# RashmikaDushan/MocapV2

Measured on AMD Instinct MI355X. Metric: frames/sec (6-cam 1080p), higher is better.
Workload: dtype u8+int64+f64; 1 GPU; 6-camera 1920x1080 synthetic IR frames, 8 markers (BASELINE.json configs[1]); cameras=6, width=1920, height=1080, markers=8, distortion=mild, frames_resident_in_hbm=True, batches_in_flight=3, resident_batches=3, status_ok=True, input=gray frames, parallelism=single launch, time-major

## Files before the change

### mocapv2_amd/csrc/abi_blob.hip

```cpp
#include "ctx.h"

static_assert(sizeof(mocap_contour) == sizeof(ContourRec), "debug record layout");

struct ScanTurn { std::mutex mu; hipEvent_t done = nullptr; bool have = false; };
static ScanTurn g_scan_turn[64];

extern "C" {

static int check_frames(mocap_ctx* c, const void* frames, int n_images, int cam_mod, int slot_base, size_t image_stride, int pitch)
{
    if (!c || !frames) return fail(MOCAP_E_INVALID, "null argument");
    if (n_images < 1) return fail(MOCAP_E_INVALID, "n_images = %d", n_images);
    if (cam_mod < 1 || slot_base < 0 || slot_base + cam_mod > c->n_slots)
        return fail(MOCAP_E_INVALID, "slots %d..%d not in 0..%d", slot_base, slot_base + cam_mod - 1, c->n_slots - 1);
    if (pitch < c->W) return fail(MOCAP_E_INVALID, "pitch %d < width %d", pitch, c->W);
    if (n_images > 1 && image_stride < (size_t)pitch * (c->H - 1) + c->W) return fail(MOCAP_E_INVALID, "image_stride too small");
    for (int s = slot_base; s < slot_base + cam_mod; s++)
        if (c->slot_state[s] == 0) return fail(MOCAP_E_STATE, "mocap_set_undistort was not called for slot %d", s);
    return 0;
}


static int excess_base(int thr_mul, int sel)
{
    int c = sel ? thr_mul - 67 : thr_mul - 154;
    if (c > thr_mul - 1) c = thr_mul - 1;
    if (c > 254) c = 254;
    return c < 0 ? 0 : c;
}

static int ensure_gray_scratch(mocap_ctx* c, size_t bytes)
{
    if (bytes <= c->gray_scratch.n) return 0;
    std::lock_guard<std::mutex> lk(c->mu);
    return c->gray_scratch.reserve(bytes);
}

static int threshold_mul(const mocap_ctx* c)
{
    const double ft = floor(c->prm.thresh);
    return ft < -1.0 ? 0 : (ft > 255.0 ? 256 : (int)ft + 1);
}

static FilterArgs filter_args(const mocap_ctx* c, const void* src, size_t image_stride, int pitch, uint32_t* mask, uint32_t* cells,
                              int slot_base, int cam_mod, int n_images, int thr_mul)
{
    const Tiling tl = tiling(c);
    FilterArgs a{};
    a.src = (const uint8_t*)src; a.image_stride = image_stride; a.pitch = pitch; a.H = c->H; a.W = c->W;
    a.mask = mask; a.words_per_row = c->wpr; a.cam_mod = cam_mod; a.cells = cells;
    a.n_images = n_images; a.n_steps = (n_images + cam_mod - 1) / cam_mod;
    a.thr_mul = thr_mul;
    a.n_strips = tl.n_strips; a.rows_per_chunk = tl.rows; a.n_cgroups = tl.n_cgroups;
    a.pipelined = c->W >= 4 && (c->W & 3) == 0 && c->H >= 2;
    if (slot_base >= 0) {
        a.map = slot_map(c, slot_base); a.mapw = slot_mapw(c, slot_base); a.map4 = slot_map4(c, slot_base);
        a.rowbox = c->rowbox ? c->rowbox + (size_t)slot_base * c->H * tl.n_strips : nullptr;
    }
    return a;
}

struct Batch {
    int n_images, cam_mod, slot_base;
    size_t image_stride; int pitch;
    uint32_t* mask; uint32_t* cells;
    bool own_mask;
    hipStream_t s;
};

static void read_probe(mocap_ctx* c, int thr_mul)
{
    if (!c->probe_pending || hipEventQuery(c->probe_ev) != hipSuccess) return;
    unsigned long long n_cur = 0, n_alt = 0;
    for (int i = 0; i < 128; i++) { n_cur += c->probe_host[PROBE_STRIDE * i]; n_alt += c->probe_host[PROBE_STRIDE * i + 1]; }
    if (c->tune.probe_debug) fprintf(stderr, "[probe] base %d: %llu hot cells, alternative %d: %llu\n", excess_base(thr_mul, c->base_sel), n_cur, excess_base(thr_mul, c->base_sel ^ 1), n_alt);
    const unsigned long long n_lo = c->base_sel == 0 ? n_cur : n_alt, n_hi = c->base_sel == 0 ? n_alt : n_cur;
    c->base_sel = (n_lo * 4 <= n_hi * 5) ? 0 : 1;
    const unsigned long long n_now = c->base_sel == 0 ? n_lo : n_hi;
    c->hot_dense = c->probe_images > 0 && n_now > 400ull * (unsigned long long)c->probe_images;
    c->probe_pending = false;
}

struct ScanBounds {
    int thr_mul;
    int fixed_base;
    int base, base_alt;
    int allow, allow_cut1, allow_cut2, allow_alt;
};
static ScanBounds scan_bounds(const mocap_ctx* c, int slot_base, int cam_mod, int thr_mul)
{
    ScanBounds b{thr_mul, c->tune.excess_base, 0, 0, -1, -1, -1, -1};
    if (b.fixed_base >= 0) { if (b.fixed_base > thr_mul - 1) b.fixed_base = thr_mul - 1; if (b.fixed_base > 254) b.fixed_base = 254; if (b.fixed_base < 0) b.fixed_base = 0; }
    b.base = b.fixed_base >= 0 ? b.fixed_base : excess_base(thr_mul, c->base_sel);
    b.base_alt = excess_base(thr_mul, c->base_sel ^ 1);
    long long wmax = 0;
    bool ok = true;
    for (int sl = slot_base; sl < slot_base + cam_mod; sl++) {
        if (c->slot_wmax[sl] == 0) ok = false;
        wmax = c->slot_wmax[sl] > wmax ? c->slot_wmax[sl] : wmax;
    }
    auto t5 = [](int n) { return (n - 1 < 2 ? n - 1 : 2) + 1; };
    auto t5full = [](int n) { return n < 5 ? n : 5; };
    const long long per_tap = 1024LL * (2LL * thr_mul - 2LL * b.base - 1), per_tap_alt = 1024LL * (2LL * thr_mul - 2LL * b.base_alt - 1);
    if (!c->tile_rows || !c->tile_cols || !c->reach || !c->cflags) ok = false;
    if (ok && wmax > 0 && per_tap > 0) {
        b.allow = (int)((per_tap * t5full(c->W) * t5full(c->H) - 1) / wmax);
        const long long taps1 = t5(c->W) * t5full(c->H) < t5full(c->W) * t5(c->H) ? t5(c->W) * t5full(c->H) : t5full(c->W) * t5(c->H);
        b.allow_cut1 = (int)((per_tap * taps1 - 1) / wmax);
        b.allow_cut2 = (int)((per_tap * t5(c->W) * t5(c->H) - 1) / wmax);
        if (per_tap_alt > 0) b.allow_alt = (int)((per_tap_alt * t5full(c->W) * t5full(c->H) - 1) / wmax);
    }
    if (!c->tune.skip_dark) b.allow = -1;
    return b;
}

struct FilterPath {
    bool remap;
    bool compact;
    bool rows_staged;
    bool direct;
    bool bayer;
    uint64_t remap_bits;
    int rows_dw;
    const void* frames;
    BayerArgs bl;
};
static int choose_path(mocap_ctx* c, const Batch& bt, const void* frames, const BayerArgs* bayer, int allow, FilterPath& p)
{
    p = FilterPath{};
    p.compact = c->W >= 8 && bt.cam_mod <= 64;
    for (int sl = bt.slot_base; sl < bt.slot_base + bt.cam_mod; sl++) {
        if (c->slot_state[sl] == 2) { p.remap = true; if (sl - bt.slot_base < 64) p.remap_bits |= 1ull << (sl - bt.slot_base); }
        if (c->slot_state[sl] == 2 && !c->slot_compact[sl]) p.compact = false;
    }
    if (c->tune.general_filter) p.compact = false;
    p.rows_staged = p.remap && c->tune.rows_staged && c->map4 && c->rowbox && (c->W & 15) == 0 && c->H >= 2;
    for (int sl = bt.slot_base; sl < bt.slot_base + bt.cam_mod; sl++)
        if (!c->slot_compact[sl]) p.rows_staged = false;
    p.rows_dw = c->tune.rows_stage_dw < 0 || c->tune.rows_stage_dw > rows_stage_dwords() ? rows_stage_dwords() : c->tune.rows_stage_dw;
    if (allow < 0 && !c->tune.dense_boxes) p.compact = false;
    p.frames = frames;
    p.bayer = bayer != nullptr;
    if (bayer) p.bl = *bayer;
    if (bayer && !bayer->dst) {
        p.direct = p.compact && allow >= 0 && bt.own_mask && bayer_scan_direct(p.bl);
        if (!p.direct) {
            const size_t bytes = (size_t)(bt.n_images - 1) * bt.image_stride + (size_t)(c->H - 1) * bt.pitch + c->W;
            TRY(ensure_gray_scratch(c, bytes));
            p.bl.dst = c->gray_scratch;
        }
        p.frames = p.direct ? (const void*)p.bl.src : (const void*)p.bl.dst;
    }
    return 0;
}

static int filter_dense(mocap_ctx* c, const Batch& bt, const FilterPath& p, int thr_mul)
{
    FilterArgs a = filter_args(c, p.frames, bt.image_stride, bt.pitch, bt.mask, bt.cells, bt.slot_base, bt.cam_mod, bt.n_images, thr_mul);
    if (!c->tune.remap_pipeline) a.pipelined = 0;
    a.staged = p.rows_staged; a.stage_dw = p.rows_dw;
    if (p.bayer) { launch_bayer_gray(p.bl, bt.s); HIP_TRY(hipGetLastError()); }
    if (bt.own_mask) c->mask_dirty = true;
    EvPair ev; bool on;
    prof_begin(c, bt.s, ev, on);
    launch_filter_mask(a, p.remap, bt.s);
    prof_end(c, PROF_FILTER, bt.s, ev, on);
    HIP_TRY(hipGetLastError());
    return 0;
}

static BoxArgs box_args(const mocap_ctx* c, const Batch& bt, const FilterPath& p, const ScanBounds& sb)
{
    const Tiling tl = tiling(c);
    BoxArgs a{};
    a.src = (const uint8_t*)p.frames; a.image_stride = bt.image_stride; a.pitch = bt.pitch; a.H = c->H; a.W = c->W;
    a.mask = bt.mask; a.words_per_row = c->wpr; a.cells = bt.cells;
    a.map4 = slot_map4(c, bt.slot_base);
    a.srcbox = c->srcbox ? c->srcbox + (size_t)bt.slot_base * source_cells(c) : nullptr;
    a.remap_bits = p.remap_bits;
    a.cam_mod = bt.cam_mod; a.n_images = bt.n_images; a.n_steps = (bt.n_images + bt.cam_mod - 1) / bt.cam_mod;
    a.thr_mul = sb.thr_mul;
    a.rows_per_chunk = tl.rows; a.n_strips = tl.n_strips; a.n_chunks = tl.n_cgroups * 4;
    const size_t tr_words = c->mask_images * cells_per_image(c) * 4;
    a.tile_rows = c->tile_rows + (c->tile_rows_flip ? tr_words : 0);
    a.tile_rows_next = c->tile_rows + (c->tile_rows_flip ? 0 : tr_words);
    a.n_clear = c->tile_rows_hold[c->tile_rows_flip ^ 1];
    a.tile_cols = c->tile_cols + (c->tile_rows_flip ? tr_words / 4 : 0);
    a.tile_cols_next = c->tile_cols + (c->tile_rows_flip ? 0 : tr_words / 4);
    a.wide_split = c->tune.wide_split == 2 || (c->tune.wide_split == 1 && !c->hot_dense);
    a.cluster = c->tune.cluster;
    a.cur_box = bt.own_mask ? c->cur_box : c->cur_box_ext;
    a.items = c->items; a.n_items = c->n_items; a.cap_items = (uint32_t)c->items.n;
    a.dense = sb.allow < 0;
    a.wide_tiles = c->wide_tiles; a.cap_wide = (uint32_t)c->wide_tiles.n; a.wide_quads_remap = c->tune.wide_quads_remap; a.wide_quads_identity = c->tune.wide_quads_identity;
    a.wide_bands = c->tune.wide_bands;
    if (c->W < 4 || p.direct) a.wide_tiles = nullptr;
    a.bayer = p.direct ? p.bl : BayerArgs{};
    a.stage_bytes = c->tune.box_stage_bytes;
    a.prio = c->tune.box_prio;
    a.ext_mask = bt.own_mask ? 0 : 1;
    return a;
}

static BrightArgs bright_args(const mocap_ctx* c, const Batch& bt, const FilterPath& p, const ScanBounds& sb, uint32_t* tile_rows, uint32_t* tile_cols,
                              bool scan_zeroes)
{
    const Tiling tl = tiling(c);
    uint64_t ncx64 = (uint64_t)((c->W + 7) / 8);
    const uint64_t ncells = ncx64 * (uint64_t)((c->H + 7) / 8);
    int wide = (c->W % 16 == 0) && (bt.pitch % 16 == 0) && (bt.image_stride % 16 == 0) && (((uintptr_t)p.frames & 15) == 0) && ncx64 >= 4;
    if (wide && ncells * (ncx64 / 2) >= (1ull << 32)) wide = 0;
    if (!c->tune.scan_wide) wide = 0;
    if (wide) ncx64 /= 2;
    const uint32_t ncx_magic = (ncx64 > 1 && ncells * ncx64 < (1ull << 32)) ? (uint32_t)(((1ull << 32) + ncx64 - 1) / ncx64) : 0u;
    BrightArgs b{(const uint8_t*)p.frames, bt.image_stride, bt.pitch, c->H, c->W, bt.n_images, bt.cam_mod, ncx_magic, wide, sb.base, sb.allow / 4, sb.allow_cut1 / 4, sb.allow_cut2 / 4,
                 c->reach + (size_t)bt.slot_base * source_cells(c), c->cflags + (size_t)bt.slot_base * source_cells(c),
                 tile_rows, tl.n_cgroups * 4, tl.n_strips, (uint32_t)(((1u << 23) + tl.rows - 1) / tl.rows),
                 bt.mask, bt.own_mask ? 0 : (size_t)bt.n_images * mask_image_words(c->H, c->wpr), ((uintptr_t)bt.mask & 15) == 0, nullptr, sb.base_alt, sb.allow_alt / 4, 0};
    b.prio = c->tune.scan_prio;
    b.max_blocks = c->tune.scan_blocks_per_cu * c->n_cu; b.blocks_x = 0;
    b.zero_counters = scan_zeroes ? c->n_items.p : nullptr;
    b.block_ctr = c->n_items + 160;
    b.slices = c->tune.scan_slices; b.image0 = 0; b.slice_images = bt.n_images;
    b.tile_cols = tile_cols;
    return b;
}

static int scan_tiles(mocap_ctx* c, const Batch& bt, const FilterPath& p, const ScanBounds& sb, uint32_t* tile_rows, uint32_t* tile_cols,
                      bool scan_zeroes, BrightArgs& b, bool& mark_after_scan)
{
    const hipStream_t s = bt.s;
    b = bright_args(c, bt, p, sb, tile_rows, tile_cols, scan_zeroes);
    const bool probe = sb.fixed_base < 0 && !c->probe_pending && sb.allow_alt >= 0 && sb.base_alt != sb.base && !p.bayer &&
                       (c->probe_age == 0 || c->probe_age >= 32);
    if (probe) {
        HIP_TRY(hipMemsetAsync(c->probe_dev, 0, PROBE_BYTES, s));
        b.probe = c->probe_dev;
    }
    c->probe_age = probe ? 1 : c->probe_age + 1;
    const bool fused = p.bayer && bt.own_mask && (p.direct || bayer_scan_fusable(p.bl));
    const bool two_step = !fused && c->hotmap && (c->tune.scan_hotmap == 2 || (c->tune.scan_hotmap == 1 && c->hot_dense));
    if (two_step) { b.hotmap = c->hotmap; b.hot_words = hot_map_words(c->H, c->W, b.wide); b.mark_grid = c->tune.mark_blocks_per_cu * c->n_cu; }
    ScanTurn* turn = c->tune.scan_serial && c->device >= 0 && c->device < 64 ? &g_scan_turn[c->device] : nullptr;
    std::unique_lock<std::mutex> turn_lock;
    if (turn) {
        turn_lock = std::unique_lock<std::mutex>(turn->mu);
        if (!turn->done) HIP_TRY(hipEventCreateWithFlags(&turn->done, hipEventDisableTiming));
        if (turn->have) HIP_TRY(hipStreamWaitEvent(s, turn->done, 0));
    }
    EvPair ev; bool on;
    prof_begin(c, s, ev, on);
    if (fused) launch_bayer_gray_scan(p.bl, b, s);
    else {
        if (p.bayer) launch_bayer_gray(p.bl, s);
        launch_bright_cells(b, s);
    }
    prof_end(c, PROF_SCAN, s, ev, on);
    HIP_TRY(hipGetLastError());
    if (turn) {
        HIP_TRY(hipEventRecord(turn->done, s));
        turn->have = true;
        turn_lock.unlock();
    }
    mark_after_scan = two_step;
    if (probe) {
        HIP_TRY(hipMemcpyAsync(c->probe_host, c->probe_dev, PROBE_BYTES, hipMemcpyDeviceToHost, s));
        HIP_TRY(hipEventRecord(c->probe_ev, s));
        c->probe_pending = true;
        c->probe_images = (bt.n_images + 15) / 16;
    }
    return 0;
}

static int settle_tiles(mocap_ctx* c, const BoxArgs& a, const BrightArgs& mark_args, bool mark_after_scan, hipStream_t s)
{
    EvPair ev; bool on;
    prof_begin(c, s, ev, on);
    if (mark_after_scan) {
        launch_mark_tiles(mark_args, s);
        HIP_TRY(hipGetLastError());
    }
    launch_settle_tiles(a, s);
    prof_end(c, PROF_SETTLE, s, ev, on);
    HIP_TRY(hipGetLastError());
    if (!a.dense) {
        if (a.n_images > c->tile_rows_hold[c->tile_rows_flip]) c->tile_rows_hold[c->tile_rows_flip] = a.n_images;
        c->tile_rows_hold[c->tile_rows_flip ^ 1] = 0;
        c->tile_rows_flip ^= 1;
    }
    return 0;
}

static int report_box_timing(mocap_ctx* c, const uint64_t* timing, hipStream_t s)
{
    std::vector<uint64_t> t((size_t)6 * c->box_grid);
    HIP_TRY(hipStreamSynchronize(s));
    HIP_TRY(hipMemcpy(t.data(), timing, sizeof(uint64_t) * t.size(), hipMemcpyDeviceToHost));
    double sum[6] = {0, 0, 0, 0, 0, 0}, mx = 0;
    for (int b = 0; b < c->box_grid; b++) {
        double tot = 0;
        for (int i = 0; i < 6; i++) { sum[i] += (double)t[6 * b + i]; if (i < 5) tot += (double)t[6 * b + i]; }
        mx = tot > mx ? tot : mx;
    }
    const double n = sum[5] > 0 ? sum[5] : 1;
    uint32_t cnt[16];
    HIP_TRY(hipMemcpy(cnt, c->n_items, sizeof(cnt), hipMemcpyDeviceToHost));
    fprintf(stderr, "[box] list: %u items, %u wide-tile entries, %u split tiles\n", cnt[0], cnt[8], cnt[SPLIT_COUNTER]);
    fprintf(stderr, "[box] items %.0f (%.1f per wave) | cycles per item: header+wait %.0f, stage %.0f, patch %.0f, threshold %.0f, majority+next %.0f | busiest wave %.0f cycles\n",
            sum[5], sum[5] / c->box_grid, sum[0] / n, sum[1] / n, sum[2] / n, sum[3] / n, sum[4] / n, mx);
    return 0;
}

static int filter_boxes(mocap_ctx* c, const Batch& bt, const FilterPath& p, BoxArgs& a)
{
    const hipStream_t s = bt.s;
    Buf<uint64_t> timing;
    if (c->tune.box_timing) {
        TRY(timing.reserve((size_t)6 * c->box_grid));
        HIP_TRY(hipMemsetAsync(timing, 0, sizeof(uint64_t) * 6 * c->box_grid, s));
    }
    a.timing = timing;
    EvPair ev; bool on;
    prof_begin(c, s, ev, on);
    const bool fork_wide = c->tune.wide_fork != 0;
    if (a.wide_tiles) {
        FilterArgs f = filter_args(c, a.src, bt.image_stride, bt.pitch, bt.mask, bt.cells, bt.slot_base, bt.cam_mod, bt.n_images, a.thr_mul);
        f.tiles = c->wide_tiles; f.n_tiles = c->n_items + 8; f.cap_tiles = a.cap_wide;
        f.staged = p.rows_staged; f.stage_dw = p.rows_dw;
        hipStream_t ws = s;
        if (fork_wide) {
            HIP_TRY(hipEventRecord(c->ev_fork, s));
            if (!c->side) HIP_TRY(hipStreamCreateWithFlags(&c->side, hipStreamNonBlocking));
            HIP_TRY(hipStreamWaitEvent(c->side, c->ev_fork, 0));
            ws = c->side;
        }
        launch_filter_tiles(f, p.remap, c->tune.wide_blocks_per_cu * c->n_cu, ws);
        HIP_TRY(hipGetLastError());
        if (fork_wide) HIP_TRY(hipEventRecord(c->ev_join, c->side));
    }
    launch_box_filter(a, c->box_grid, s, p.direct);
    HIP_TRY(hipGetLastError());
    if (a.wide_tiles && fork_wide) HIP_TRY(hipStreamWaitEvent(s, c->ev_join, 0));
    prof_end(c, PROF_FILTER, s, ev, on);
    return timing ? report_box_timing(c, timing, s) : 0;
}

static int run_filter(mocap_ctx* c, const void* frames, int n_images, int cam_mod, int slot_base, size_t image_stride,
                      int pitch, uint32_t* mask, uint32_t* cells, hipStream_t s, const BayerArgs* bayer = nullptr)
{
    const Batch bt{n_images, cam_mod, slot_base, image_stride, pitch, mask, cells, mask == c->mask, s};
    c->walk_count_zeroed = false;
    if (cells == c->cells) c->last_images = n_images;
    const int thr_mul = threshold_mul(c);
    read_probe(c, thr_mul);
    const ScanBounds sb = scan_bounds(c, slot_base, cam_mod, thr_mul);
    FilterPath p;
    TRY(choose_path(c, bt, frames, bayer, sb.allow, p));
    if (!p.compact) return filter_dense(c, bt, p, thr_mul);
    if (bt.own_mask && c->mask_dirty) {
        HIP_TRY(hipMemsetAsync(c->mask, 0, sizeof(uint32_t) * c->mask_images * mask_image_words(c->H, c->wpr), s));
        std::vector<uint32_t> init(c->mask_images * cells_per_image(c) * 4);
        for (size_t i = 0; i < init.size(); i += 4) { init[i] = 1u; init[i + 1] = 1u; init[i + 2] = 1u; init[i + 3] = 1u; }
        HIP_TRY(hipStreamSynchronize(s));
        HIP_TRY(hipMemcpy(c->cur_box, init.data(), sizeof(uint32_t) * init.size(), hipMemcpyHostToDevice));
        c->mask_dirty = false;
    }
    BoxArgs a = box_args(c, bt, p, sb);
    if ((size_t)n_images * cells_per_image(c) * BOX_MAX_PARTS > c->items.n) return fail(MOCAP_E_STATE, "work list smaller than the batch");
    const bool scan_zeroes = !a.dense && !p.bayer && c->tune.scan_blocks_per_cu == 0 && c->tune.scan_slices <= 1;
    if (!scan_zeroes) HIP_TRY(hipMemsetAsync(c->n_items, 0, 1024, s));
    a.zero8 = bt.own_mask ? c->walk_count.p : nullptr;
    c->walk_count_zeroed = a.zero8 != nullptr;
    BrightArgs mark_args{}; bool mark_after_scan = false;
    if (!a.dense) TRY(scan_tiles(c, bt, p, sb, a.tile_rows, const_cast<uint32_t*>(a.tile_cols), scan_zeroes, mark_args, mark_after_scan));
    else if (p.bayer) {
        launch_bayer_gray(p.bl, s);
        HIP_TRY(hipGetLastError());
    }
    TRY(settle_tiles(c, a, mark_args, mark_after_scan, s));
    return filter_boxes(c, bt, p, a);
}

static const uint32_t* contour_boxes(mocap_ctx* c)
{
    return (c->mask_dirty || !c->tune.contour_boxes) ? nullptr : c->cur_box;
}

static int ensure_contour_work(mocap_ctx* c, size_t n_images)
{
    if (n_images <= c->cwork_images) return 0;
    std::lock_guard<std::mutex> lk(c->mu);
    if (n_images <= c->cwork_images) return 0;
    c->cwork_images = 0;
    int rc = c->cwork.reserve(contour_work_bytes() * n_images);
    if (!rc) rc = c->walk_list.reserve((contour_walk_bytes() * n_images + 7) / 8);
    if (!rc) rc = c->link_list.reserve(((contour_link_bytes() + sizeof(uint32_t)) * n_images + 7) / 8);
    if (!rc) rc = c->walk_count.reserve(64);
    if (rc) { c->cwork.release(); c->walk_list.release(); c->link_list.release(); return rc; }
    c->cwork_images = n_images;
    return 0;
}

static int report_follow_timing(const uint64_t* follow_dbg, int follow_grid, hipStream_t s)
{
    std::vector<uint64_t> t((size_t)8 * follow_grid);
    HIP_TRY(hipStreamSynchronize(s));
    HIP_TRY(hipMemcpy(t.data(), follow_dbg, sizeof(uint64_t) * t.size(), hipMemcpyDeviceToHost));
    double sum[8] = {0, 0, 0, 0, 0, 0, 0, 0}, mx[3] = {0, 0, 0}, mxsteps = 0; int used = 0;
    for (int b = 0; b < follow_grid; b++) {
        if (t[8 * b + 5] == 0) continue;
        used++;
        for (int i = 0; i < 8; i++) sum[i] += (double)t[8 * b + i];
        for (int i = 0; i < 3; i++) mx[i] = (double)t[8 * b + i] > mx[i] ? (double)t[8 * b + i] : mx[i];
        mxsteps = (double)t[8 * b + 3] > mxsteps ? (double)t[8 * b + 3] : mxsteps;
    }
    const double u = used ? used : 1;
    fprintf(stderr, "[follow] %d of %d waves had work | per wave (mean / max us): store %.1f / %.1f, refill %.1f / %.1f, walk %.1f / %.1f | wave steps %.0f (max %.0f), "
                    "lanes alive per step %.1f, walks %.1f, refills %.1f | us per wave step %.3f\n",
            used, follow_grid, sum[0] / u / 100, mx[0] / 100, sum[1] / u / 100, mx[1] / 100, sum[2] / u / 100, mx[2] / 100, sum[3] / u, mxsteps,
            sum[3] > 0 ? sum[4] / sum[3] : 0.0, sum[5] / u, sum[6] / u, sum[3] > 0 ? sum[2] / 100 / sum[3] : 0.0);
    return 0;
}

static int report_contour_timing(const uint64_t* timing, int n_images, hipStream_t s)
{
    std::vector<uint64_t> t((size_t)8 * n_images);
    HIP_TRY(hipStreamSynchronize(s));
    HIP_TRY(hipMemcpy(t.data(), timing, sizeof(uint64_t) * t.size(), hipMemcpyDeviceToHost));
    double sum[4] = {0, 0, 0, 0}, mx = 0; uint64_t lo = ~0ull, hi = 0;
    for (int i = 0; i < n_images; i++) {
        for (int k = 0; k < 4; k++) sum[k] += (double)(t[8 * i + k + 1] - t[8 * i + k]);
        double tot = (double)(t[8 * i + 4] - t[8 * i]); mx = tot > mx ? tot : mx;
        lo = t[8 * i] < lo ? t[8 * i] : lo; hi = t[8 * i + 4] > hi ? t[8 * i + 4] : hi;
    }
    {
        int worst = 0; double wt = 0, sc = 0, ss = 0;
        for (int i = 0; i < n_images; i++) {
            double tot = (double)(t[8 * i + 4] - t[8 * i]);
            if (tot > wt) { wt = tot; worst = i; }
            sc += (double)t[8 * i + 5]; ss += (double)t[8 * i + 6];
        }
        fprintf(stderr, "[contours] slowest image %d: %.1f us, candidates %llu, longest border %llu steps, borders %llu | mean candidates %.1f, mean longest border %.1f steps\n",
                worst, wt / 100, (unsigned long long)t[8 * worst + 5], (unsigned long long)t[8 * worst + 6], (unsigned long long)t[8 * worst + 7],
                sc / n_images, ss / n_images);
    }
    fprintf(stderr, "[contours] mean us per block: candidates %.1f follow %.1f link %.1f order %.1f | slowest block %.1f | first start to last end %.1f\n",
            sum[0] / n_images / 100, sum[1] / n_images / 100, sum[2] / n_images / 100, sum[3] / n_images / 100, mx / 100, (double)(hi - lo) / 100);
    return 0;
}

static int run_contours(mocap_ctx* c, const uint32_t* mask, const uint32_t* cells, const uint32_t* boxes, int n_images, int32_t* out_xy, long xy_stride,
                        int32_t* out_count, long count_stride, int max_blobs, mocap_contour* dbg, int32_t* dbg_count, int dbg_cap, hipStream_t s)
{
    ContourArgs a;
    a.mask = mask; a.words_per_row = c->wpr; a.H = c->H; a.W = c->W; a.n_images = n_images;
    a.out_xy = out_xy; a.out_count = out_count; a.max_blobs = max_blobs;
    a.xy_stride = xy_stride; a.count_stride = count_stride;
    a.min_area = c->prm.min_area; a.min_circ = c->prm.min_circ;
    a.dbg = (ContourRec*)dbg; a.dbg_count = dbg_count; a.dbg_cap = dbg_cap;
    long long ms = 4LL * c->H * c->W + 16;
    a.max_steps = ms > (1 << 22) ? (1 << 22) : (int)ms;
    Tiling tl = tiling(c);
    a.cells = cells; a.boxes = boxes; a.rows_per_chunk = tl.rows; a.n_chunks = tl.n_cgroups * 4; a.n_strips = tl.n_strips;
    if ((long long)a.n_chunks * a.n_strips * ((tl.rows + 7) / 8) > 65535 || c->wpr > 4096) a.cells = nullptr;
    TRY(ensure_contour_work(c, n_images));
    a.work = c->cwork;
    const bool split = c->tune.contours_split != 0;
    a.walk_list = split ? c->walk_list : nullptr; a.link_list = c->link_list; a.walk_count = c->walk_count;
    a.follow_grid = c->n_cu * 4;
    a.follow_grid2 = c->n_cu;
    a.image_grid = c->tune.contour_blocks_per_cu * c->n_cu;
    a.counters_zeroed = mask == c->mask && c->walk_count_zeroed;
    c->walk_count_zeroed = false;
    a.defer_links = c->tune.contour_defer == 2 || (c->tune.contour_defer == 1 && c->hot_dense);
    a.wait_list = (uint32_t*)((uint8_t*)c->link_list.p + contour_link_bytes() * c->cwork_images);
    a.follow_list = 0; a.tree_pass = 0; a.follow_dbg_list = c->tune.follow_timing == 2 ? 1 : 0;
    Buf<uint64_t> follow_dbg, timing;
    if (c->tune.follow_timing && split) {
        TRY(follow_dbg.reserve((size_t)8 * a.follow_grid));
        HIP_TRY(hipMemsetAsync(follow_dbg, 0, sizeof(uint64_t) * 8 * a.follow_grid, s));
    }
    a.follow_dbg = follow_dbg;
    a.prio = c->tune.contour_prio;
    if (c->tune.contour_timing) {
        TRY(timing.reserve((size_t)8 * n_images));
        HIP_TRY(hipMemsetAsync(timing, 0, sizeof(uint64_t) * 8 * n_images, s));
    }
    a.timing = timing;
    EvPair p; bool on;
    prof_begin(c, s, p, on);
    launch_contours(a, s);
    prof_end(c, PROF_CONTOURS, s, p, on);
    HIP_TRY(hipGetLastError());
    if (follow_dbg) TRY(report_follow_timing(follow_dbg, a.follow_grid, s));
    if (timing) TRY(report_contour_timing(timing, n_images, s));
    return 0;
}

static int grow_mask_group(mocap_ctx* c, size_t n_images)
{
    const size_t tiles = n_images * cells_per_image(c);
    TRY(c->mask.reserve(n_images * mask_image_words(c->H, c->wpr), true));
    TRY(c->cells.reserve(tiles, true));
    std::vector<uint32_t> init(tiles * 4);
    for (size_t i = 0; i < init.size(); i += 2) { init[i] = 0xffffffffu; init[i + 1] = 0u; }
    TRY(c->tile_rows.reserve(2 * init.size()));
    HIP_TRY(hipMemcpy(c->tile_rows, init.data(), sizeof(uint32_t) * init.size(), hipMemcpyHostToDevice));
    HIP_TRY(hipMemcpy(c->tile_rows + init.size(), init.data(), sizeof(uint32_t) * init.size(), hipMemcpyHostToDevice));
    TRY(c->tile_cols.reserve(2 * tiles));
    HIP_TRY(hipMemset(c->tile_cols, 0, sizeof(uint32_t) * 2 * tiles));
    const int hw0 = hot_map_words(c->H, c->W, 0), hw1 = hot_map_words(c->H, c->W, 1);
    TRY(c->hotmap.reserve(n_images * (hw0 > hw1 ? hw0 : hw1), true));
    for (size_t i = 0; i < init.size(); i++) init[i] = 1u;
    TRY(c->cur_box.reserve(init.size()));
    HIP_TRY(hipMemcpy(c->cur_box, init.data(), sizeof(uint32_t) * init.size(), hipMemcpyHostToDevice));
    const size_t cap = tiles * BOX_MAX_PARTS;
    if (cap > 0xffffffffull) return fail(MOCAP_E_UNSUPPORTED, "batch too large for the work list");
    TRY(c->items.reserve(cap));
    return c->wide_tiles.reserve(4 * tiles);
}
static int ensure_mask(mocap_ctx* c, int n_images)
{
    if ((size_t)n_images <= c->mask_images) return 0;
    std::lock_guard<std::mutex> lk(c->mu);
    if ((size_t)n_images <= c->mask_images) return 0;
    c->mask_images = 0; c->last_images = 0;
    if (int rc = grow_mask_group(c, n_images)) {
        c->mask.release(); c->cells.release(); c->tile_rows.release(); c->tile_cols.release(); c->hotmap.release(); c->cur_box.release();
        c->items.release(); c->wide_tiles.release();
        return rc;
    }
    c->tile_rows_flip = 0; c->tile_rows_hold[0] = c->tile_rows_hold[1] = 0;
    c->mask_dirty = false;
    c->mask_images = n_images;
    return 0;
}

static int ensure_blocked(mocap_ctx* c, Buf<uint32_t>& m, int n_images)
{
    const size_t words = (size_t)n_images * mask_image_words(c->H, c->wpr);
    if (words <= m.n) return 0;
    std::lock_guard<std::mutex> lk(c->mu);
    return m.reserve(words, true);
}

static int ensure_ext(mocap_ctx* c, int n_images)
{
    if ((size_t)n_images <= c->cells_ext_images) return 0;
    std::lock_guard<std::mutex> lk(c->mu);
    if ((size_t)n_images <= c->cells_ext_images) return 0;
    c->cells_ext_images = 0;
    int rc = c->cells_ext.reserve((size_t)n_images * cells_per_image(c));
    if (!rc) rc = c->cur_box_ext.reserve(4 * (size_t)n_images * cells_per_image(c));
    if (rc) { c->cells_ext.release(); c->cur_box_ext.release(); return rc; }
    c->cells_ext_images = n_images;
    return 0;
}

int mocap_filter_mask(mocap_ctx_t c, const void* frames, int n_images, int cam_mod, int slot_base, size_t image_stride,
                      int pitch, uint32_t* mask_dev, void* stream)
{
    TRY(check_frames(c, frames, n_images, cam_mod, slot_base, image_stride, pitch));
    if (!mask_dev) return fail(MOCAP_E_INVALID, "null mask");
    if (set_device(c)) return MOCAP_E_HIP;
    TRY(ensure_mask(c, n_images));
    TRY(ensure_ext(c, n_images));
    TRY(ensure_blocked(c, c->mask_out, n_images));
    TRY(run_filter(c, frames, n_images, cam_mod, slot_base, image_stride, pitch, c->mask_out, c->cells_ext, (hipStream_t)stream));
    launch_mask_convert(c->mask_out, mask_dev, n_images, c->H, c->wpr, false, (hipStream_t)stream);
    HIP_TRY(hipGetLastError());
    return MOCAP_OK;
}

int mocap_contours_from_mask(mocap_ctx_t c, const uint32_t* mask_dev, int n_images, int32_t* out_xy, long xy_stride,
                             int32_t* out_count, long count_stride, int max_blobs, mocap_contour* dbg, int32_t* dbg_count,
                             int dbg_cap, void* stream)
{
    if (!c || !mask_dev || !out_xy || !out_count) return fail(MOCAP_E_INVALID, "null argument");
    if (n_images < 1 || max_blobs < 1 || xy_stride < 2L * max_blobs || count_stride < 1)
        return fail(MOCAP_E_INVALID, "n_images=%d max_blobs=%d strides %ld %ld", n_images, max_blobs, xy_stride, count_stride);
    if ((dbg != nullptr) != (dbg_count != nullptr) || (dbg && dbg_cap < 1)) return fail(MOCAP_E_INVALID, "inconsistent debug buffers");
    if (set_device(c)) return MOCAP_E_HIP;
    TRY(ensure_blocked(c, c->mask_in, n_images));
    launch_mask_convert(mask_dev, c->mask_in, n_images, c->H, c->wpr, true, (hipStream_t)stream);
    HIP_TRY(hipGetLastError());
    return run_contours(c, c->mask_in, nullptr, nullptr, n_images, out_xy, xy_stride, out_count, count_stride, max_blobs, dbg, dbg_count, dbg_cap,
                        (hipStream_t)stream);
}

int mocap_blob_centroids(mocap_ctx_t c, const void* frames, int n_images, int cam_mod, int slot_base, size_t image_stride,
                         int pitch, int32_t* out_xy, long xy_stride, int32_t* out_count, long count_stride, int max_blobs,
                         void* stream)
{
    TRY(check_frames(c, frames, n_images, cam_mod, slot_base, image_stride, pitch));
    if (!out_xy || !out_count || max_blobs < 1 || xy_stride < 2L * max_blobs || count_stride < 1)
        return fail(MOCAP_E_INVALID, "bad output arguments");
    if (set_device(c)) return MOCAP_E_HIP;
    TRY(ensure_mask(c, n_images));
    TRY(run_filter(c, frames, n_images, cam_mod, slot_base, image_stride, pitch, c->mask, c->cells, (hipStream_t)stream));
    return run_contours(c, c->mask, c->cells, contour_boxes(c), n_images, out_xy, xy_stride, out_count, count_stride, max_blobs, nullptr, nullptr, 0,
                        (hipStream_t)stream);
}

static int bayer_args(BayerArgs& a, const void* bayer, void* gray, int n_images, int H, int W, long spitch, long dpitch,
                      size_t src_image_stride, size_t dst_image_stride, int pattern, int gray_shift, bool gray_optional = false)
{
    if (!bayer || (!gray && !gray_optional)) return fail(MOCAP_E_INVALID, "null argument");
    if (n_images < 1 || n_images > 65535 || H < 3 || W < 3 || spitch < W || dpitch < W)
        return fail(MOCAP_E_INVALID, "bad geometry: n=%d H=%d W=%d pitches %ld %ld (H, W >= 3)", n_images, H, W, spitch, dpitch);
    if (n_images > 1 && (src_image_stride < (size_t)spitch * (H - 1) + W || dst_image_stride < (size_t)dpitch * (H - 1) + W))
        return fail(MOCAP_E_INVALID, "image strides smaller than an image");
    if (pattern < 0 || pattern > 3 || (gray_shift != 14 && gray_shift != 15))
        return fail(MOCAP_E_INVALID, "pattern %d (0..3 = BG, GB, RG, GR) / gray_shift %d (14 or 15)", pattern, gray_shift);
    a = BayerArgs{};
    a.src = (const uint8_t*)bayer; a.dst = (uint8_t*)gray;
    a.H = H; a.W = W; a.n_images = n_images;
    a.spitch = spitch; a.dpitch = dpitch; a.sstride = src_image_stride; a.dstride = dst_image_stride;
    a.ry = pattern >= 2; a.rx = pattern == 1 || pattern == 2;
    a.cb = gray_shift == 14 ? 1868u : 3735u; a.cg = gray_shift == 14 ? 9617u : 19235u; a.cr = gray_shift == 14 ? 4899u : 9798u;
    a.shift = gray_shift;
    return 0;
}

int mocap_blob_centroids_bayer(mocap_ctx_t c, const void* bayer_frames, void* gray_frames, int n_images, int cam_mod, int slot_base,
                               size_t image_stride, int pitch, int pattern, int gray_shift, int32_t* out_xy, long xy_stride,
                               int32_t* out_count, long count_stride, int max_blobs, void* stream)
{
    TRY(check_frames(c, bayer_frames, n_images, cam_mod, slot_base, image_stride, pitch));
    if (!out_xy || !out_count || max_blobs < 1 || xy_stride < 2L * max_blobs || count_stride < 1)
        return fail(MOCAP_E_INVALID, "bad output arguments");
    BayerArgs b;
    TRY(bayer_args(b, bayer_frames, gray_frames, n_images, c->H, c->W, pitch, pitch, image_stride, image_stride, pattern, gray_shift, true));
    if (set_device(c)) return MOCAP_E_HIP;
    TRY(ensure_mask(c, n_images));
    TRY(run_filter(c, gray_frames, n_images, cam_mod, slot_base, image_stride, pitch, c->mask, c->cells, (hipStream_t)stream, &b));
    return run_contours(c, c->mask, c->cells, contour_boxes(c), n_images, out_xy, xy_stride, out_count, count_stride, max_blobs, nullptr, nullptr, 0,
                        (hipStream_t)stream);
}

int mocap_refine_centroids(mocap_ctx_t c, const void* frames, int n_images, int cam_mod, int slot_base, size_t image_stride, int pitch,
                           int pattern, int gray_shift, const int32_t* xy, long xy_stride, const int32_t* count, long count_stride,
                           int max_blobs, int radius, int floor_, int iters, int coords, double* out_xy, long out_xy_stride,
                           int32_t* out_info, long out_info_stride, void* stream)
{
    if (!c || !frames || !xy || !count || !out_xy) return fail(MOCAP_E_INVALID, "null argument");
    if (radius < 1 || radius > 31 || floor_ < 0 || floor_ > 254 || iters < 1 || iters > 8 || (coords != 0 && coords != 1))
        return fail(MOCAP_E_INVALID, "radius %d (1..31), floor %d (0..254), iters %d (1..8), coords %d (0 raw, 1 ideal)", radius, floor_, iters, coords);
    if (max_blobs < 1 || max_blobs > SUBPIX_MAX_BLOBS || xy_stride < 2L * max_blobs || count_stride < 1 || out_xy_stride < 2L * max_blobs ||
        (out_info && out_info_stride < 2L * max_blobs))
        return fail(MOCAP_E_INVALID, "max_blobs %d (1..%d), strides %ld %ld %ld %ld", max_blobs, SUBPIX_MAX_BLOBS, xy_stride, count_stride,
                    out_xy_stride, out_info_stride);
    if (pattern < -1 || pattern > 3 || (pattern >= 0 && gray_shift != 14 && gray_shift != 15))
        return fail(MOCAP_E_INVALID, "pattern %d (-1 = gray frames, 0..3 = BG, GB, RG, GR) / gray_shift %d (14 or 15)", pattern, gray_shift);
    if (pattern >= 0 && (c->H < 3 || c->W < 3)) return fail(MOCAP_E_INVALID, "Bayer frames need H, W >= 3");
    TRY(check_frames(c, frames, n_images, cam_mod, slot_base, image_stride, pitch));
    if (set_device(c)) return MOCAP_E_HIP;
    RefineArgs a{};
    a.src = (const uint8_t*)frames; a.image_stride = image_stride; a.pitch = pitch; a.H = c->H; a.W = c->W;
    a.n_images = n_images; a.cam_mod = cam_mod;
    if (pattern >= 0) {
        BayerArgs b;
        TRY(bayer_args(b, frames, nullptr, n_images, c->H, c->W, pitch, pitch, image_stride, image_stride, pattern, gray_shift, true));
        a.bayer = 1; a.ry = b.ry; a.rx = b.rx; a.cb = b.cb; a.cg = b.cg; a.cr = b.cr; a.shift = b.shift;
    }
    a.lens = c->lens + (size_t)SUBPIX_LENS * slot_base;
    a.xy = xy; a.xy_stride = xy_stride; a.count = count; a.count_stride = count_stride; a.max_blobs = max_blobs;
    a.radius = radius; a.floor = floor_; a.iters = iters; a.coords = coords;
    a.out_xy = out_xy; a.out_xy_stride = out_xy_stride; a.out_info = out_info; a.out_info_stride = out_info_stride;
    launch_refine_centroids(a, (hipStream_t)stream);
    HIP_TRY(hipGetLastError());
    return MOCAP_OK;
}

int mocap_undistort_u8(mocap_ctx_t c, int slot, const void* src, void* dst, int spitch, int dpitch, void* stream)
{
    if (!c || !src || !dst) return fail(MOCAP_E_INVALID, "null argument");
    if (slot < 0 || slot >= c->n_slots || c->slot_state[slot] == 0) return fail(MOCAP_E_STATE, "undistort slot %d not set", slot);
    if (spitch < c->W || dpitch < c->W) return fail(MOCAP_E_INVALID, "pitch < width");
    if (set_device(c)) return MOCAP_E_HIP;
    launch_undistort((const uint8_t*)src, (uint8_t*)dst, c->H, c->W, spitch, dpitch, slot_map(c, slot), slot_mapw(c, slot), (hipStream_t)stream);
    HIP_TRY(hipGetLastError());
    return MOCAP_OK;
}

int mocap_image_filter_u8(mocap_ctx_t c, const void* src, void* dst, int spitch, int dpitch, int order, int slot, void* stream)
{
    if (!c || !src || !dst) return fail(MOCAP_E_INVALID, "null argument");
    if (order != 0 && order != 1) return fail(MOCAP_E_INVALID, "order must be 0 (image_filter_gpu) or 1 (image_filter_cpu)");
    if (spitch < c->W || dpitch < c->W) return fail(MOCAP_E_INVALID, "pitch < width");
    if (slot >= c->n_slots || (slot >= 0 && c->slot_state[slot] == 0)) return fail(MOCAP_E_STATE, "undistort slot %d not set", slot);
    if (set_device(c)) return MOCAP_E_HIP;
    hipStream_t s = (hipStream_t)stream;
    const int thr_mul = threshold_mul(c), ithresh = thr_mul - 1;
    if (order == 1) {
        const uint8_t* in = (const uint8_t*)src;
        int ip = spitch;
        if (slot >= 0 && c->slot_state[slot] == 2) {
            return fail(MOCAP_E_UNSUPPORTED, "image_filter_cpu order with undistortion: call mocap_undistort_u8 first");
        }
        launch_median5(in, (uint8_t*)dst, c->H, c->W, ip, dpitch, ithresh, 1, s);
        HIP_TRY(hipGetLastError());
        return MOCAP_OK;
    }
    TRY(ensure_mask(c, 1));
    const FilterArgs a = filter_args(c, src, 0, spitch, c->mask, c->cells, slot, 1, 1, thr_mul);
    c->mask_dirty = true; c->last_images = 1;
    launch_filter_mask(a, slot >= 0 && c->slot_state[slot] == 2, s);
    HIP_TRY(hipGetLastError());
    launch_mask_expand(c->mask, c->wpr, (uint8_t*)dst, c->H, c->W, dpitch, s);
    HIP_TRY(hipGetLastError());
    return MOCAP_OK;
}

int mocap_box_blur_u8(mocap_ctx_t c, const void* src, void* dst, int H, int W, int spitch, int dpitch, int ksize, void* stream)
{
    if (!c || !src || !dst) return fail(MOCAP_E_INVALID, "null argument");
    if (H < 1 || W < 1 || spitch < W || dpitch < W || ksize < 1 || ksize > 31) return fail(MOCAP_E_INVALID, "bad geometry");
    if (set_device(c)) return MOCAP_E_HIP;
    launch_box_blur((const uint8_t*)src, (uint8_t*)dst, H, W, spitch, dpitch, ksize, (hipStream_t)stream);
    HIP_TRY(hipGetLastError());
    return MOCAP_OK;
}

int mocap_bayer_gray_u8(mocap_ctx_t c, const void* bayer, void* gray, int n_images, int H, int W, long spitch, long dpitch,
                        size_t src_image_stride, size_t dst_image_stride, int pattern, int gray_shift, void* stream)
{
    if (!c) return fail(MOCAP_E_INVALID, "null argument");
    BayerArgs a;
    TRY(bayer_args(a, bayer, gray, n_images, H, W, spitch, dpitch, src_image_stride, dst_image_stride, pattern, gray_shift));
    if (set_device(c)) return MOCAP_E_HIP;
    launch_bayer_gray(a, (hipStream_t)stream);
    HIP_TRY(hipGetLastError());
    return MOCAP_OK;
}

int mocap_demosaic_u8(mocap_ctx_t c, const void* bayer, void* bgr, int H, int W, int spitch, void* stream)
{
    if (!c || !bayer || !bgr) return fail(MOCAP_E_INVALID, "null argument");
    if (H < 1 || W < 1 || spitch < W) return fail(MOCAP_E_INVALID, "bad geometry");
    if (set_device(c)) return MOCAP_E_HIP;
    launch_demosaic((const uint8_t*)bayer, (uint8_t*)bgr, H, W, spitch, (hipStream_t)stream);
    HIP_TRY(hipGetLastError());
    return MOCAP_OK;
}

int mocap_tile_stats(mocap_ctx_t c, uint64_t* tiles, uint64_t* skipped)
{
    if (!c) return fail(MOCAP_E_INVALID, "null context");
    if (set_device(c)) return MOCAP_E_HIP;
    uint64_t total = 0, full = 0;
    if (c->cells && c->last_images > 0) {
        HIP_TRY(hipDeviceSynchronize());
        Tiling t = tiling(c);
        size_t per = cells_per_image(c), n = per * (size_t)c->last_images;
        std::vector<uint32_t> w(n);
        HIP_TRY(hipMemcpy(w.data(), c->cells, sizeof(uint32_t) * n, hipMemcpyDeviceToHost));
        int valid_chunks = (c->H + t.rows - 1) / t.rows;
        total = (uint64_t)c->last_images * valid_chunks * t.n_strips;
        for (size_t i = 0; i < n; i++) full += w[i] >> 31;
    }
    if (tiles) *tiles = total;
    if (skipped) *skipped = total - full;
    return MOCAP_OK;
}

int mocap_list_stats(mocap_ctx_t c, uint32_t* items, uint32_t* wide, uint32_t* split)
{
    if (!c) return fail(MOCAP_E_INVALID, "null context");
    if (set_device(c)) return MOCAP_E_HIP;
    uint32_t cnt[16] = {0};
    static_assert(SPLIT_COUNTER != 0 && SPLIT_COUNTER != 8 && SPLIT_COUNTER < 16, "a word of its own in the first line of the counter block");
    if (c->n_items) {
        HIP_TRY(hipDeviceSynchronize());
        HIP_TRY(hipMemcpy(cnt, c->n_items, sizeof(cnt), hipMemcpyDeviceToHost));
    }
    if (items) *items = cnt[0];
    if (wide) *wide = cnt[8];
    if (split) *split = cnt[SPLIT_COUNTER];
    return MOCAP_OK;
}

}
```

### mocapv2_amd/csrc/bayer_gray.hip

```cpp
#include <hip/hip_runtime.h>
#include <stdint.h>
#include "kernels.h"
#include "scan_mark.h"
#include "bayer.h"

namespace mocap {

__device__ __forceinline__ uint32_t wave_prev(uint32_t v) { return (uint32_t)__builtin_amdgcn_update_dpp(0, (int)v, 0x138, 0xf, 0xf, true); }
__device__ __forceinline__ uint32_t wave_next(uint32_t v) { return (uint32_t)__builtin_amdgcn_update_dpp(0, (int)v, 0x130, 0xf, 0xf, true); }

template <int ND> struct RowPairs { uint32_t e[ND], o[ND], Le[ND], Ro[ND]; };

template <int ND, bool NEED_LE, bool NEED_RO>
__device__ __forceinline__ RowPairs<ND> row_pairs(const uint32_t (&w)[ND])
{
    RowPairs<ND> r;
#pragma unroll
    for (int i = 0; i < ND; i++) {
        r.e[i] = prm(0, w[i], 0x0c020c00u);
        r.o[i] = prm(0, w[i], 0x0c030c01u);
    }
    if (NEED_LE) {
        const uint32_t pw = wave_prev(w[ND - 1]);
        r.Le[0] = prm(pw, w[0], 0x0c010c07u);
#pragma unroll
        for (int i = 1; i < ND; i++) r.Le[i] = prm(w[i], w[i - 1], 0x0c050c03u);
    }
    if (NEED_RO) {
        const uint32_t nw = wave_next(w[0]);
#pragma unroll
        for (int i = 0; i < ND - 1; i++) r.Ro[i] = prm(w[i + 1], w[i], 0x0c040c02u);
        r.Ro[ND - 1] = prm(nw, w[ND - 1], 0x0c040c02u);
    }
    return r;
}

template <int ND> struct LaneLoad;
template <> struct LaneLoad<2> { typedef uint2 type; };
template <> struct LaneLoad<4> { typedef uint4 type; };

template <int ND>
__global__ __launch_bounds__(256) void bayer_gray_kernel(BayerArgs a)
{
    constexpr int PX = 4 * ND, WAVE_PX = 62 * PX;
    typedef typename LaneLoad<ND>::type vec_t;
    const int lane = threadIdx.x;
    const int y = __builtin_amdgcn_readfirstlane(blockIdx.y * 4 + threadIdx.y);
    if (y >= a.H) return;
    const int x0 = blockIdx.x * WAVE_PX - PX + PX * lane;
    const int yc = y < 1 ? 1 : (y > a.H - 2 ? a.H - 2 : y);
    const uint8_t* __restrict__ src = a.src + (size_t)blockIdx.z * a.sstride + (size_t)(yc - 1) * a.spitch;
    const bool in = x0 >= 0 && x0 < a.W;
    const uint32_t off = in ? (uint32_t)x0 : 0u;
    uint32_t wu[ND], wc[ND], wd[ND];
    {
        const vec_t vu = *(const vec_t*)(src + off), vc = *(const vec_t*)(src + a.spitch + off), vd = *(const vec_t*)(src + 2 * a.spitch + off);
        __builtin_memcpy(wu, &vu, sizeof(vu)); __builtin_memcpy(wc, &vc, sizeof(vc)); __builtin_memcpy(wd, &vd, sizeof(vd));
    }
    if (!in) {
#pragma unroll
        for (int i = 0; i < ND; i++) wu[i] = wc[i] = wd[i] = 0u;
    }

    const bool red_row = (yc & 1) == a.ry;
    const bool even_is_colour = (red_row ? a.rx : 1 - a.rx) == 0;
    const uint32_t cx = red_row ? a.cr : a.cb, cy = red_row ? a.cb : a.cr;
    const LumaCoef k{cx, a.cg, cy, cx << 16, a.cg << 16, cy << 16, 1u << (a.shift - 1), a.shift};

    uint32_t g[PX];
    const RowPairs<ND> C = row_pairs<ND, true, true>(wc);
    if (even_is_colour) {
        const RowPairs<ND> U = row_pairs<ND, true, false>(wu), D = row_pairs<ND, true, false>(wd);
#pragma unroll
        for (int i = 0; i < ND; i++) {
            luma2(C.e[i], mean4(C.Le[i], C.o[i], U.e[i], D.e[i]), mean4(U.Le[i], U.o[i], D.Le[i], D.o[i]), k, g[4 * i], g[4 * i + 2]);
            luma2(mean2(C.e[i], C.Ro[i]), C.o[i], mean2(U.o[i], D.o[i]), k, g[4 * i + 1], g[4 * i + 3]);
        }
    } else {
        const RowPairs<ND> U = row_pairs<ND, false, true>(wu), D = row_pairs<ND, false, true>(wd);
#pragma unroll
        for (int i = 0; i < ND; i++) {
            luma2(mean2(C.Le[i], C.o[i]), C.e[i], mean2(U.e[i], D.e[i]), k, g[4 * i], g[4 * i + 2]);
            luma2(C.o[i], mean4(C.e[i], C.Ro[i], U.o[i], D.o[i]), mean4(U.e[i], U.Ro[i], D.e[i], D.Ro[i]), k, g[4 * i + 1], g[4 * i + 3]);
        }
    }
    if (x0 == 0) g[0] = g[1];
    if (x0 + PX == a.W) g[PX - 1] = g[PX - 2];
    if (in && lane >= 1 && lane <= 62) {
        uint32_t out[ND];
#pragma unroll
        for (int i = 0; i < ND; i++) out[i] = g[4 * i] | (g[4 * i + 1] << 8) | (g[4 * i + 2] << 16) | (g[4 * i + 3] << 24);
        vec_t v;
        __builtin_memcpy(&v, out, sizeof(v));
        *(vec_t*)(a.dst + (size_t)blockIdx.z * a.dstride + (size_t)y * a.dpitch + x0) = v;
    }
}

__device__ __forceinline__ LumaCoef luma_coef(const BayerArgs& a, bool red_row)
{
    const uint32_t cx = red_row ? a.cr : a.cb, cy = red_row ? a.cb : a.cr;
    return LumaCoef{cx, a.cg, cy, cx << 16, a.cg << 16, cy << 16, 1u << (a.shift - 1), a.shift};
}

template <bool WRITE>
__global__ __launch_bounds__(256) void bayer_gray_scan_kernel(BayerArgs a, BrightArgs b)
{
    constexpr int ND = 4, PX = 16, WAVE_PX = 62 * PX;
    const int lane = threadIdx.x;
    const int cy = __builtin_amdgcn_readfirstlane(blockIdx.y * 4 + threadIdx.y);
    if (8 * cy >= a.H) return;
    const int image = blockIdx.z;
    const int x0 = blockIdx.x * WAVE_PX - PX + PX * lane;
    const bool in = x0 >= 0 && x0 < a.W;
    const uint32_t off = in ? (uint32_t)x0 : 0u;
    const uint8_t* __restrict__ src = a.src + (size_t)image * a.sstride;
    uint8_t* __restrict__ dst = a.dst + (size_t)image * a.dstride;

    const bool red0 = a.ry == 0, red1 = a.ry == 1;
    const bool eic0 = (red0 ? a.rx : 1 - a.rx) == 0, eic1 = (red1 ? a.rx : 1 - a.rx) == 0;
    const LumaCoef k0 = luma_coef(a, red0), k1 = luma_coef(a, red1);

    auto load_row = [&](int r) {
        r = r < 0 ? 0 : (r > a.H - 1 ? a.H - 1 : r);
        uint4 v = *(const uint4*)(src + (size_t)r * a.spitch + off);
        if (!in) v = make_uint4(0u, 0u, 0u, 0u);
        return v;
    };
    auto pairs_of = [&](uint4 v) {
        uint32_t w[ND];
        __builtin_memcpy(w, &v, sizeof(v));
        return row_pairs<ND, true, true>(w);
    };
    uint4 raw[10];
#pragma unroll
    for (int r = 0; r < 10; r++) raw[r] = load_row(8 * cy - 1 + r);

    RowPairs<ND> U = pairs_of(raw[0]), C = pairs_of(raw[1]);
    uint32_t acc0 = 0, acc1 = 0;
    const bool writer = in && lane >= 1 && lane <= 62;
#pragma unroll
    for (int j = 0; j < 8; j++) {
        const int y = 8 * cy + j;
        const RowPairs<ND> D = pairs_of(raw[j + 2]);
        if (y != 0 && y != a.H - 1) {
            const bool eic = (j & 1) ? eic1 : eic0;
            const LumaCoef& k = (j & 1) ? k1 : k0;
            uint32_t g[PX];
            if (eic) {
#pragma unroll
                for (int i = 0; i < ND; i++) {
                    luma2(C.e[i], mean4(C.Le[i], C.o[i], U.e[i], D.e[i]), mean4(U.Le[i], U.o[i], D.Le[i], D.o[i]), k, g[4 * i], g[4 * i + 2]);
                    luma2(mean2(C.e[i], C.Ro[i]), C.o[i], mean2(U.o[i], D.o[i]), k, g[4 * i + 1], g[4 * i + 3]);
                }
            } else {
#pragma unroll
                for (int i = 0; i < ND; i++) {
                    luma2(mean2(C.Le[i], C.o[i]), C.e[i], mean2(U.e[i], D.e[i]), k, g[4 * i], g[4 * i + 2]);
                    luma2(C.o[i], mean4(C.e[i], C.Ro[i], U.o[i], D.o[i]), mean4(U.e[i], U.Ro[i], D.e[i], D.Ro[i]), k, g[4 * i + 1], g[4 * i + 3]);
                }
            }
            if (x0 == 0) g[0] = g[1];
            if (x0 + PX == a.W) g[PX - 1] = g[PX - 2];
            uint4 out;
            out.x = g[0] | (g[1] << 8) | (g[2] << 16) | (g[3] << 24);
            out.y = g[4] | (g[5] << 8) | (g[6] << 16) | (g[7] << 24);
            out.z = g[8] | (g[9] << 8) | (g[10] << 16) | (g[11] << 24);
            out.w = g[12] | (g[13] << 8) | (g[14] << 16) | (g[15] << 24);
            const bool twice = y == 1 || y == a.H - 2;
            if (WRITE && writer) {
                *(uint4*)(dst + (size_t)y * a.dpitch + x0) = out;
                if (y == 1) *(uint4*)(dst + x0) = out;
                if (y == a.H - 2) *(uint4*)(dst + (size_t)(a.H - 1) * a.dpitch + x0) = out;
            }
            const uint32_t base4 = (uint32_t)b.base * 0x01010101u, c8 = 8u * (uint32_t)b.base;
            const uint32_t e0 = excess2_row(out.x, out.y, base4, c8), e1 = excess2_row(out.z, out.w, base4, c8);
            acc0 += twice ? 2u * e0 : e0;
            acc1 += twice ? 2u * e1 : e1;
        }
        U = C; C = D;
    }
    if (writer) {
        const int ncx = a.W >> 3, n = ncx * (a.H >> 3);
        const int slot = image % b.cam_mod;
        const uint2* __restrict__ reach = b.reach + (size_t)slot * n;
        const uint8_t* __restrict__ cflags = b.cflags + (size_t)slot * n;
        uint32_t* __restrict__ rows = b.tile_rows + (size_t)image * b.n_chunks * b.n_strips * 4;
        uint32_t* __restrict__ cols = b.tile_cols + (size_t)image * b.n_chunks * b.n_strips;
        const int ci = cy * ncx + (x0 >> 3);
        mark_hot_cell(b, reach, cflags, rows, cols, ci, acc0);
        mark_hot_cell(b, reach, cflags, rows, cols, ci + 1, acc1);
    }
}

__global__ __launch_bounds__(256) void bayer_gray_any_kernel(BayerArgs a)
{
    const int x = blockIdx.x * 64 + threadIdx.x, y = blockIdx.y * 4 + threadIdx.y;
    if (x >= a.W || y >= a.H) return;
    const int yc = y < 1 ? 1 : (y > a.H - 2 ? a.H - 2 : y), xc = x < 1 ? 1 : (x > a.W - 2 ? a.W - 2 : x);
    const uint8_t* __restrict__ p = a.src + (size_t)blockIdx.z * a.sstride + (size_t)yc * a.spitch + xc;
    const long sp = a.spitch;
    a.dst[(size_t)blockIdx.z * a.dstride + (size_t)y * a.dpitch + x] =
        (uint8_t)site_gray(p[0], p[-1], p[1], p[-sp], p[sp], p[-sp - 1], p[-sp + 1], p[sp - 1], p[sp + 1], (yc & 1) == a.ry,
                           (xc & 1) == a.rx, a);
}

void launch_bayer_gray(const BayerArgs& a, hipStream_t s)
{
    auto aligned = [&](int n) {
        return a.W % n == 0 && a.spitch % n == 0 && a.dpitch % n == 0 && a.sstride % n == 0 && a.dstride % n == 0 &&
               (uintptr_t)a.src % n == 0 && (uintptr_t)a.dst % n == 0;
    };
    if (aligned(16))
        hipLaunchKernelGGL(bayer_gray_kernel<4>, dim3((a.W + 62 * 16 - 1) / (62 * 16), (a.H + 3) / 4, a.n_images), dim3(64, 4), 0, s, a);
    else if (aligned(8))
        hipLaunchKernelGGL(bayer_gray_kernel<2>, dim3((a.W + 62 * 8 - 1) / (62 * 8), (a.H + 3) / 4, a.n_images), dim3(64, 4), 0, s, a);
    else
        hipLaunchKernelGGL(bayer_gray_any_kernel, dim3((a.W + 63) / 64, (a.H + 3) / 4, a.n_images), dim3(64, 4), 0, s, a);
}

bool bayer_scan_direct(const BayerArgs& a)
{
    return a.W % 16 == 0 && a.H % 8 == 0 && a.H >= 8 && a.spitch % 16 == 0 && a.sstride % 16 == 0 && (uintptr_t)a.src % 16 == 0;
}

bool bayer_scan_fusable(const BayerArgs& a)
{
    return bayer_scan_direct(a) && a.dpitch % 16 == 0 && a.dstride % 16 == 0 && (uintptr_t)a.dst % 16 == 0;
}

void launch_bayer_gray_scan(const BayerArgs& a, const BrightArgs& b, hipStream_t s)
{
    const dim3 grid((a.W + 62 * 16 - 1) / (62 * 16), (a.H / 8 + 3) / 4, a.n_images);
    if (a.dst) hipLaunchKernelGGL(bayer_gray_scan_kernel<true>, grid, dim3(64, 4), 0, s, a, b);
    else hipLaunchKernelGGL(bayer_gray_scan_kernel<false>, grid, dim3(64, 4), 0, s, a, b);
}

}
```

### mocapv2_amd/csrc/blob_scan.hip

```cpp
#include <hip/hip_runtime.h>
#include <stdint.h>
#include "kernels.h"
#include "scan_mark.h"

namespace mocap {

__device__ __forceinline__ uint4 load_once16(const uint8_t* p)
{
    typedef unsigned int u32x4 __attribute__((ext_vector_type(4)));
    const u32x4 q = __builtin_nontemporal_load((const u32x4*)p);
    return make_uint4(q.x, q.y, q.z, q.w);
}

template <bool WIDE, bool FULL, bool MAP>
__device__ __forceinline__ void bright_cells_block(const BrightArgs& a, const int bx, const int image)
{
    const int ncx = (a.W + 7) >> 3, ncy = (a.H + 7) >> 3, n = ncx * ncy;
    const uint8_t* __restrict__ img = a.src + (size_t)image * a.image_stride;
    uint2 v[2][8];
    int ci[2], cr[2];
    uint32_t sh[2];
    bool in_range[2];
    if (WIDE) {
        const int half = ncx >> 1, np = half * ncy;
        int p = bx * 256 + threadIdx.x;
        in_range[0] = in_range[1] = p < np;
        p = p < np ? p : np - 1;
        const int row = (int)__umulhi((uint32_t)p, a.ncx_magic), cxp = p - row * half;
        cr[0] = cr[1] = row;
        ci[0] = row * ncx + 2 * cxp; ci[1] = ci[0] + 1;
        sh[0] = sh[1] = 0;
        if (FULL) {
            const uint32_t off0 = (uint32_t)(8 * row) * (uint32_t)a.pitch + 16u * (uint32_t)cxp;
#pragma unroll
            for (int j = 0; j < 8; j++) {
                const uint4 q = load_once16(img + (off0 + (uint32_t)(j * a.pitch)));
                v[0][j] = make_uint2(q.x, q.y); v[1][j] = make_uint2(q.z, q.w);
            }
        } else {
#pragma unroll
            for (int j = 0; j < 8; j++) {
                int r = 8 * row + j;
                r = r < a.H ? r : a.H - 1;
                const uint4 q = load_once16(img + ((uint32_t)r * (uint32_t)a.pitch + 16u * (uint32_t)cxp));
                v[0][j] = make_uint2(q.x, q.y); v[1][j] = make_uint2(q.z, q.w);
            }
        }
    } else {
        const int i0 = bx * 512 + threadIdx.x;
#pragma unroll
        for (int u = 0; u < 2; u++) {
            int i = i0 + 256 * u;
            in_range[u] = i < n;
            i = i < n ? i : n - 1;
            ci[u] = i;
            cr[u] = a.ncx_magic ? (int)__umulhi((uint32_t)i, a.ncx_magic) : i / ncx;
            const int cx = i - cr[u] * ncx;
            const int c = 8 * cx, cc = c < a.W - 8 ? c : a.W - 8;
            sh[u] = (uint32_t)(8 * (c - cc));
#pragma unroll
            for (int j = 0; j < 8; j++) {
                int r = 8 * cr[u] + j;
                r = r < a.H ? r : a.H - 1;
                __builtin_memcpy(&v[u][j], img + ((uint32_t)r * (uint32_t)a.pitch + (uint32_t)cc), 8);
            }
        }
    }
    const int slot = image % a.cam_mod;
    const uint2* __restrict__ reach = a.reach + (size_t)slot * n;
    const uint8_t* __restrict__ cflags = a.cflags + (size_t)slot * n;
    uint32_t* __restrict__ rows = a.tile_rows + (size_t)image * a.n_chunks * a.n_strips * 4;
    uint32_t* __restrict__ cols = a.tile_cols + (size_t)image * a.n_chunks * a.n_strips;
    const uint32_t base4 = (uint32_t)a.base * 0x01010101u, c8 = 8u * (uint32_t)a.base;
    uint32_t level[2] = {0u, 0u}, sum[2];
#pragma unroll
    for (int u = 0; u < 2; u++) {
        uint32_t acc = 0;
#pragma unroll
        for (int j = 0; j < 8; j++) {
            if (WIDE) {
                const uint32_t e2 = excess2_row(v[u][j].x, v[u][j].y, base4, c8);
                if (FULL || 8 * cr[u] + j < a.H) acc += e2;
            } else {
                uint64_t vv = (((uint64_t)v[u][j].y << 32) | v[u][j].x) >> sh[u];
                const uint32_t e2 = excess2_row((uint32_t)vv, (uint32_t)(vv >> 32), base4, c8);
                if (8 * cr[u] + j < a.H) acc += e2;
            }
        }
        if (MAP) level[u] = in_range[u] ? hot_level(a, acc) : 0u;
        sum[u] = acc;
        if (a.probe && (image & 15) == 0) {
            const uint32_t alt4 = (uint32_t)a.base_alt * 0x01010101u, alt8 = 8u * (uint32_t)a.base_alt;
            uint32_t acc2 = 0;
#pragma unroll
            for (int j = 0; j < 8; j++) {
                const uint64_t vv = WIDE ? (((uint64_t)v[u][j].y << 32) | v[u][j].x) : ((((uint64_t)v[u][j].y << 32) | v[u][j].x) >> sh[u]);
                const uint32_t e2 = excess2_row((uint32_t)vv, (uint32_t)(vv >> 32), alt4, alt8);
                if (FULL || 8 * cr[u] + j < a.H) acc2 += e2;
            }
            const int n_cur = __popcll(__ballot((int)acc > a.hot)), n_alt = __popcll(__ballot((int)acc2 > a.hot_alt));
            if ((threadIdx.x & 63) == 0) {
                atomicAdd(&a.probe[PROBE_STRIDE * (bx & 127)], (uint32_t)n_cur);
                atomicAdd(&a.probe[PROBE_STRIDE * (bx & 127) + 1], (uint32_t)n_alt);
            }
        }
    }
    if (!MAP) {
        mark_hot_cell(a, reach, cflags, rows, cols, ci[0], sum[0]);
        mark_hot_cell(a, reach, cflags, rows, cols, ci[1], sum[1]);
    }
    if (MAP) {
        const int lane = threadIdx.x & 63;
        uint32_t* __restrict__ hm = a.hotmap + (size_t)image * a.hot_words;
        if (WIDE) {
            uint32_t w = (level[0] | (level[1] << 2)) << (4 * (lane & 7));
            w |= (uint32_t)__builtin_amdgcn_update_dpp(0, (int)w, 0xB1 , 0xf, 0xf, true);
            w |= (uint32_t)__builtin_amdgcn_update_dpp(0, (int)w, 0x4E , 0xf, 0xf, true);
            w |= (uint32_t)__builtin_amdgcn_update_dpp(0, (int)w, 0x141 , 0xf, 0xf, true);
            if ((lane & 7) == 0 && w != 0u) hm[(bx * 256 + (int)threadIdx.x) >> 3] = w;
        } else {
#pragma unroll
            for (int u = 0; u < 2; u++) {
                uint32_t w = level[u] << (2 * (lane & 15));
                w |= (uint32_t)__builtin_amdgcn_update_dpp(0, (int)w, 0xB1, 0xf, 0xf, true);
                w |= (uint32_t)__builtin_amdgcn_update_dpp(0, (int)w, 0x4E, 0xf, 0xf, true);
                w |= (uint32_t)__builtin_amdgcn_update_dpp(0, (int)w, 0x141, 0xf, 0xf, true);
                w |= (uint32_t)__builtin_amdgcn_update_dpp(0, (int)w, 0x140 , 0xf, 0xf, true);
                if ((lane & 15) == 0 && w != 0u) hm[(bx * 512 + (int)threadIdx.x + 256 * u) >> 4] = w;
            }
        }
    }
}

__global__ __launch_bounds__(256) void mark_tiles_kernel(BrightArgs a)
{
    __shared__ uint16_t s_list[4][1024];
    __shared__ uint32_t s_tab[4][32][6];
    const int lane = threadIdx.x & 63, wv = threadIdx.x >> 6;
    const int wpi = (a.hot_words + 255) >> 8;
    const int n_cells = ((a.W + 7) >> 3) * ((a.H + 7) >> 3);
    for (long long piece = (long long)blockIdx.x * 4 + wv; piece < (long long)wpi * a.n_images; piece += (long long)gridDim.x * 4) {
    const int image = (int)(piece / wpi), wave_word0 = (int)(piece - (long long)image * wpi) * 256;
    uint32_t* __restrict__ hm = a.hotmap + (size_t)image * a.hot_words;
    uint32_t wk[4];
#pragma unroll
    for (int k = 0; k < 4; k++) {
        const int wi = wave_word0 + 64 * k + lane;
        wk[k] = wi < a.hot_words ? hm[wi] : 0u;
    }
    if (__ballot((wk[0] | wk[1] | wk[2] | wk[3]) != 0u) == 0ull) continue;
#pragma unroll
    for (int k = 0; k < 4; k++)
        if (wk[k] != 0u) hm[wave_word0 + 64 * k + lane] = 0u;
    uint32_t (*tab)[6] = s_tab[wv];
    if (lane < 32) { tab[lane][0] = 0xffffffffu; tab[lane][1] = 0xffffffffu; tab[lane][2] = 0u; tab[lane][3] = 0xffffffffu; tab[lane][4] = 0u; tab[lane][5] = 0u; }
    const int slot = image % a.cam_mod;
    const uint2* __restrict__ reach = a.reach + (size_t)slot * n_cells;
    const uint8_t* __restrict__ cflags = a.cflags + (size_t)slot * n_cells;
    uint32_t* __restrict__ rows = a.tile_rows + (size_t)image * a.n_chunks * a.n_strips * 4;
    uint32_t* __restrict__ cols = a.tile_cols + (size_t)image * a.n_chunks * a.n_strips;
    auto widen = [&](int t, uint32_t ya, uint32_t yb, uint32_t xa, uint32_t xb, uint32_t m) __attribute__((always_inline)) {
        const uint4 cur = *(const uint4*)(rows + 4 * t);
        const uint32_t have = cols[t];
        if (!(cur.x <= ya && cur.y >= yb && cur.z <= xa && cur.w >= xb)) {
            atomicMin(&rows[4 * t], ya);
            atomicMax(&rows[4 * t + 1], yb);
            atomicMin(&rows[4 * t + 2], xa);
            atomicMax(&rows[4 * t + 3], xb);
        }
        if ((have & m) != m) atomicOr(&cols[t], m);
    };
#pragma unroll 1
    for (int k = 0; k < 4; k++) {
        const uint32_t w = k == 0 ? wk[0] : (k == 1 ? wk[1] : (k == 2 ? wk[2] : wk[3]));
        const uint32_t nz = (w | (w >> 1)) & 0x55555555u;
        const int cnt = __popc(nz);
        if (__ballot(cnt != 0) == 0ull) continue;
        const int word0 = wave_word0 + 64 * k;
        int incl = cnt;
#pragma unroll
        for (int d = 1; d < 64; d <<= 1) {
            const int o = __shfl_up(incl, d);
            if (lane >= d) incl += o;
        }
        const int total = __builtin_amdgcn_readlane(incl, 63);
        int at = incl - cnt;
        for (uint32_t m = nz; m; m &= m - 1) {
            const int j2 = __ffs((int)m) - 1;
            s_list[wv][at++] = (uint16_t)((lane << 6) | (j2 << 1) | ((w >> j2) & 3u));
        }
        __builtin_amdgcn_s_waitcnt(0xc07f);
        __builtin_amdgcn_wave_barrier();
        for (int e0 = 0; e0 < total; e0 += 64) {
            const int e = e0 + lane;
            if (e < total) {
                const uint32_t v = s_list[wv][e];
                const int ci = 16 * (word0 + (int)(v >> 6)) + (int)((v >> 2) & 15u);
                if (ci < n_cells) {
                    const uint2 rc = reach[ci];
                    const int x0 = (int)(rc.x & 0xffffu), x1 = (int)(rc.x >> 16), y0 = (int)(rc.y & 0xffffu), y1 = (int)(rc.y >> 16);
                    if (x0 <= x1 && level_is_hot(v & 3u, cflags[ci])) {
                        const int xa = x0 - 4 > 0 ? x0 - 4 : 0, xb = x1 + 4 < a.W - 1 ? x1 + 4 : a.W - 1;
                        const int ya = y0 - 4 > 0 ? y0 - 4 : 0, yb = y1 + 4 < a.H - 1 ? y1 + 4 : a.H - 1;
                        const int ch0 = (int)(((uint32_t)ya * a.rows_magic) >> 23), ch1 = (int)(((uint32_t)yb * a.rows_magic) >> 23);
                        const int st0 = (int)(((uint32_t)xa * 34953u) >> 23), st1 = (int)(((uint32_t)xb * 34953u) >> 23);
                        for (int ch = ch0; ch <= ch1; ch++)
                            for (int st = st0; st <= st1; st++) {
                                const int t = ch * a.n_strips + st, q = t & 31;
                                const uint32_t m = tile_col_bits(st, xa, xb);
                                const uint32_t old = atomicCAS(&tab[q][0], 0xffffffffu, (uint32_t)t);
                                if (old == 0xffffffffu || old == (uint32_t)t) {
                                    atomicMin(&tab[q][1], (uint32_t)ya); atomicMax(&tab[q][2], (uint32_t)yb);
                                    atomicMin(&tab[q][3], (uint32_t)xa); atomicMax(&tab[q][4], (uint32_t)xb);
                                    atomicOr(&tab[q][5], m);
                                } else
                                    widen(t, (uint32_t)ya, (uint32_t)yb, (uint32_t)xa, (uint32_t)xb, m);
                            }
                    }
                }
            }
        }
        __builtin_amdgcn_s_waitcnt(0xc07f);
        __builtin_amdgcn_wave_barrier();
    }
    if (lane < 32 && tab[lane][0] != 0xffffffffu) widen((int)tab[lane][0], tab[lane][1], tab[lane][2], tab[lane][3], tab[lane][4], tab[lane][5]);
    __builtin_amdgcn_s_waitcnt(0xc07f);
    __builtin_amdgcn_wave_barrier();
    }
}

template <bool WIDE, bool FULL = false, bool MAP = true>
__global__ __launch_bounds__(256) void bright_cells_kernel(BrightArgs a)
{
    if (a.prio == 1) __builtin_amdgcn_s_setprio(1);
    else if (a.prio == 2) __builtin_amdgcn_s_setprio(2);
    else if (a.prio == 3) __builtin_amdgcn_s_setprio(3);
    const uint32_t total = (uint32_t)a.blocks_x * (uint32_t)a.slice_images;
    if (a.zero_counters && blockIdx.x == 0) a.zero_counters[threadIdx.x] = 0u;
    if (a.block_ctr == nullptr) {
        for (uint32_t vb = blockIdx.x; vb < total; vb += gridDim.x) {
            const uint32_t image = vb / (uint32_t)a.blocks_x;
            bright_cells_block<WIDE, FULL, MAP>(a, (int)(vb - image * (uint32_t)a.blocks_x), a.image0 + (int)image);
        }
    } else {
        __shared__ uint32_t s_next[2];
        constexpr uint32_t CH = 16;
        uint32_t v0 = blockIdx.x * CH;
        for (int it = 0; v0 < total; it++) {
            if (threadIdx.x == 0) s_next[it & 1] = gridDim.x * CH + atomicAdd(a.block_ctr, CH);
            for (uint32_t vb = v0; vb < v0 + CH && vb < total; vb++) {
                const uint32_t image = vb / (uint32_t)a.blocks_x;
                bright_cells_block<WIDE, FULL, MAP>(a, (int)(vb - image * (uint32_t)a.blocks_x), a.image0 + (int)image);
            }
            __syncthreads();
            v0 = s_next[it & 1];
        }
    }
    if (a.mask_words) {
        const size_t nthreads = (size_t)gridDim.x * 256;
        const size_t g = (size_t)blockIdx.x * 256 + threadIdx.x;
        if (a.mask_aligned16) {
            const size_t quads = a.mask_words >> 2;
            for (size_t q = g; q < quads; q += nthreads) ((uint4*)a.mask)[q] = make_uint4(0u, 0u, 0u, 0u);
            if (g < (a.mask_words & 3)) a.mask[(quads << 2) + g] = 0u;
        } else {
            for (size_t q = g; q < a.mask_words; q += nthreads) a.mask[q] = 0u;
        }
    }
}

void launch_bright_cells(const BrightArgs& a_, hipStream_t s)
{
    BrightArgs a = a_;
    const int n = ((a.W + 7) >> 3) * ((a.H + 7) >> 3);
    a.blocks_x = a.wide ? (n / 2 + 255) / 256 : (n + 511) / 512;
    const int slices = a.slices > 1 ? (a.slices < a.n_images ? a.slices : a.n_images) : 1;
    const int per = (a.n_images + slices - 1) / slices;
    const size_t mask_words = a.mask_words;
    for (int i0 = 0; i0 < a.n_images; i0 += per) {
        a.image0 = i0;
        a.slice_images = a.n_images - i0 < per ? a.n_images - i0 : per;
        a.mask_words = i0 == 0 ? mask_words : 0;
        const long long total = (long long)a.blocks_x * a.slice_images;
        long long grid = total;
        uint32_t* const ctr = a_.block_ctr;
        a.block_ctr = nullptr;
        if (a.max_blocks > 0 && a.max_blocks < grid) {
            grid = a.max_blocks;
            a.block_ctr = ctr ? ctr + (i0 / per) : nullptr;
        }
        if (grid > 0x7fffffffLL) grid = 0x7fffffffLL;
        const dim3 g((unsigned)grid), b(256);
        if (a.hotmap) {
            if (a.wide && a.H % 8 == 0) hipLaunchKernelGGL((bright_cells_kernel<true, true, true>), g, b, 0, s, a);
            else if (a.wide) hipLaunchKernelGGL((bright_cells_kernel<true, false, true>), g, b, 0, s, a);
            else hipLaunchKernelGGL((bright_cells_kernel<false, false, true>), g, b, 0, s, a);
        } else {
            if (a.wide && a.H % 8 == 0) hipLaunchKernelGGL((bright_cells_kernel<true, true, false>), g, b, 0, s, a);
            else if (a.wide) hipLaunchKernelGGL((bright_cells_kernel<true, false, false>), g, b, 0, s, a);
            else hipLaunchKernelGGL((bright_cells_kernel<false, false, false>), g, b, 0, s, a);
        }
    }
}
int hot_map_words(int H, int W, int wide)
{
    const int n = ((W + 7) >> 3) * ((H + 7) >> 3);
    return 32 * (wide ? (n / 2 + 255) / 256 : (n + 511) / 512);
}
void launch_mark_tiles(const BrightArgs& a, hipStream_t s)
{
    long long grid = ((long long)((a.hot_words + 255) >> 8) * a.n_images + 3) / 4;
    if (a.mark_grid > 0 && a.mark_grid < grid) grid = a.mark_grid;
    hipLaunchKernelGGL(mark_tiles_kernel, dim3((unsigned)grid), dim3(256), 0, s, a);
}

}
```

### mocapv2_amd/csrc/blob_settle.hip

```cpp
#include <hip/hip_runtime.h>
#include <stdint.h>
#include "kernels.h"

namespace mocap {

namespace {
__device__ __forceinline__ int imin(int a, int b) { return a < b ? a : b; }
__device__ __forceinline__ int imax(int a, int b) { return a > b ? a : b; }
}

__device__ __forceinline__ void choose_split(int nb, int h, int& nx, int& ny)
{
    int best = 0x7fffffff;
    nx = 1; ny = 1;
    for (int cx = 1; cx <= 4; cx++) {
        const int pb = (nb + cx - 1) / cx, Q = 2 * pb + 2;
        if (Q > 64) continue;
        const int rpw = 64 / Q, mr = BOX_HCAP / Q - 8;
        if (mr < 1) continue;
        const int cy = (h + mr - 1) / mr;
        if (cx * cy > BOX_MAX_PARTS) continue;
        const int ph = (h + cy - 1) / cy;
        const int cost = cx * cy * ((ph + 8 + rpw - 1) / rpw + 8);
        if (cost < best) { best = cost; nx = cx; ny = cy; }
    }
}

namespace {

struct Rect { int x0, x1, y0, y1; };
constexpr uint4 NO_BOX = {0xffffffffu, 0u, 0xffffffffu, 0u};

struct TileOfThread { int image, chunk, strip; size_t idx; bool valid; };
__device__ __forceinline__ TileOfThread tile_of_thread(const BoxArgs& a, int n_all)
{
    const int steps_all = (n_all + a.cam_mod - 1) / a.cam_mod;
    const long long total = (long long)a.n_chunks * a.n_strips * a.cam_mod * steps_all;
    const long long i = (long long)blockIdx.x * 256 + threadIdx.x;
    TileOfThread t{0, 0, 0, 0, i < total};
    if (t.valid) {
        const int step = (int)(i % steps_all);
        const long long rest = i / steps_all;
        const int slot = (int)(rest % a.cam_mod), tile = (int)(rest / a.cam_mod);
        t.image = step * a.cam_mod + slot;
        t.chunk = tile / a.n_strips; t.strip = tile - t.chunk * a.n_strips;
        t.valid = t.chunk * a.rows_per_chunk < a.H;
    }
    t.idx = ((size_t)t.image * a.n_chunks + t.chunk) * a.n_strips + t.strip;
    return t;
}

__device__ __forceinline__ bool scan_box(const BoxArgs& a, const TileOfThread& t, bool valid, Rect& box)
{
    box = {0, a.W - 1, 0, a.H - 1};
    if (!valid || a.dense) return valid;
    const uint4 raw = *(const uint4*)(a.tile_rows + 4 * t.idx);
    if (raw.x > raw.y) return false;
    box = {(int)raw.z, (int)raw.w, (int)raw.x, (int)raw.y};
    return true;
}

__device__ __forceinline__ bool cluster_decision(const BoxArgs& a, const TileOfThread& t, Rect& cover, Rect& exact)
{
    const int c0 = t.chunk & ~1, s0 = t.strip & ~1;
    int n_marked = 0, first = -1;
    Rect u{0x7fffffff, -1, 0x7fffffff, -1};
    for (int k = 0; k < 4; k++) {
        const int cy = c0 + (k >> 1), sx = s0 + (k & 1);
        if (cy >= a.n_chunks || sx >= a.n_strips || cy * a.rows_per_chunk >= a.H) continue;
        const uint4 o = *(const uint4*)(a.tile_rows + 4 * (((size_t)t.image * a.n_chunks + cy) * a.n_strips + sx));
        if (o.x > o.y) continue;
        if (first < 0) first = k;
        n_marked++;
        u.y0 = imin(u.y0, (int)o.x); u.y1 = imax(u.y1, (int)o.y); u.x0 = imin(u.x0, (int)o.z); u.x1 = imax(u.x1, (int)o.w);
    }
    if (n_marked < 2) return true;
    const int bx_lo = 240 * s0, bx_hi = imin(240 * (s0 + 2) - 1, a.W - 1), by_lo = c0 * a.rows_per_chunk, by_hi = imin((c0 + 2) * a.rows_per_chunk, a.H) - 1;
    const Rect e{imax(u.x0, bx_lo) & ~7, imin(u.x1 | 7, bx_hi), imax(u.y0, by_lo), imin(u.y1, by_hi)};
    if (((e.x1 - e.x0 + 8) >> 3) > 13 || e.y1 - e.y0 + 1 > 100) return true;
    cover = e; exact = u;
    return first == ((t.chunk - c0) * 2 + (t.strip - s0));
}

__device__ __forceinline__ bool record_region(const BoxArgs& a, const TileOfThread& t, bool marked, const Rect& out, const Rect& box, uint32_t& prev_x,
                                              uint32_t& prev_y)
{
    const uint32_t out_x = span_pack(out.x0, out.x1), out_y = span_pack(out.y0, out.y1);
    uint4* cb = (uint4*)(a.cur_box + 4 * t.idx);
    bool need_clear = false;
    if (!a.ext_mask) {
        const uint4 prev = *cb;
        prev_x = prev.x; prev_y = prev.y;
        const int px0 = span_first(prev.x), px1 = span_last(prev.x), py0 = span_first(prev.y), py1 = span_last(prev.y);
        if (px0 <= px1) need_clear = !(marked && out.x0 <= px0 && px1 <= out.x1 && out.y0 <= py0 && py1 <= out.y1);
        if (prev.x != out_x || prev.y != out_y || marked) *cb = tile_box_pack(out_x, out_y, box.x0, box.x1, box.y0, box.y1);
        if (a.cells[t.idx] != 0u) a.cells[t.idx] = 0u;
    } else {
        *cb = tile_box_pack(out_x, out_y, box.x0, box.x1, box.y0, box.y1);
        a.cells[t.idx] = 0u;
    }
    return need_clear;
}
__device__ __forceinline__ void clear_previous(const BoxArgs& a, bool need_clear, uint32_t prev_x, uint32_t prev_y, int image)
{
    const int lane = threadIdx.x & 63;
    for (uint64_t todo = __ballot(need_clear); todo; todo &= todo - 1) {
        const int src = __ffsll((long long)todo) - 1;
        const uint32_t cx = (uint32_t)__builtin_amdgcn_readlane((int)prev_x, src), cy = (uint32_t)__builtin_amdgcn_readlane((int)prev_y, src);
        const int cimage = __builtin_amdgcn_readlane(image, src);
        const int x0 = span_first(cx), x1 = span_last(cx), y0 = span_first(cy), y1 = span_last(cy);
        uint8_t* m = (uint8_t*)(a.mask + (size_t)cimage * mask_image_words(a.H, a.words_per_row));
        const int b0 = x0 >> 3, nr = y1 - y0 + 1, n = nr * ((x1 >> 3) - b0 + 1);
        for (int i = lane; i < n; i += 64) {
            const int bc = i / nr;
            m[mask_byte_index(y0 + (i - bc * nr), b0 + bc, a.words_per_row)] = 0;
        }
    }
}

__device__ __forceinline__ void emit_wide(const BoxArgs& a, bool wide, int image, int tile, int y0, int y1)
{
    const uint64_t wb = __ballot(wide);
    if (!wb) return;
    const int lane = threadIdx.x & 63, nbands = a.wide_bands;
    uint32_t base = 0;
    if (lane == 0) base = atomicAdd(a.n_items + 8, (uint32_t)(__popcll(wb) * nbands));
    base = (uint32_t)__builtin_amdgcn_readfirstlane((int)base);
    const uint32_t o = base + (uint32_t)(__popcll(wb & ((1ull << lane) - 1ull)) * nbands);
    if (!wide) return;
    const int hb = (y1 - y0 + nbands) / nbands;
    for (int b = 0; b < nbands; b++) {
        const int b0 = y0 + b * hb, b1 = imin(b0 + hb - 1, y1);
        if (o + b < a.cap_wide) a.wide_tiles[o + b] = wide_tile_pack(image, tile, b0, b1);
    }
}

__device__ __forceinline__ void count_split(const BoxArgs& a, bool split)
{
    const uint64_t sb = __ballot(split);
    if (sb && (threadIdx.x & 63) == 0) atomicAdd(a.n_items + SPLIT_COUNTER, (uint32_t)__popcll(sb));
}

__device__ __forceinline__ uint64_t piece_pack(int b0, int b1, int nx, int ny) { return (uint64_t)(b0 | b1 << 5 | nx << 10 | ny << 13); }

__device__ __forceinline__ int split_at_gaps(uint32_t cols, int b0, int b1, int h, int limit, uint64_t& pieces)
{
    uint32_t w = cols & ((2u << b1) - (1u << b0));
    int n = 0, parts = 0;
    pieces = 0;
    while (w) {
        const int r0 = __ffs((int)w) - 1;
        const uint32_t up = w + (1u << r0);
        const int r1 = (up ? __ffs((int)up) - 1 : 32) - 1;
        w &= up;
        int nx, ny;
        choose_split(r1 - r0 + 1, h, nx, ny);
        if (n == BOX_MAX_PARTS || 2 * (r1 - r0 + 1) + 2 * nx >= limit) return 0;
        pieces |= piece_pack(r0, r1, nx, ny) << (16 * n);
        n++; parts += nx * ny;
    }
    return (n >= 2 && parts <= BOX_MAX_PARTS) ? n : 0;
}

__device__ __forceinline__ void emit_items(const BoxArgs& a, int n_pieces, uint64_t pieces, bool split, int image, int tile, const Rect& cover,
                                           const Rect& exact, int tile_x0, int tile_x1)
{
    static_assert(BOX_MAX_PARTS <= 4, "a thread's pieces are packed into one 64-bit word");
    const int lane = threadIdx.x & 63;
    int cnt = 0;
    for (int k = 0; k < n_pieces; k++) cnt += (int)((pieces >> (16 * k + 10)) & 7u) * (int)((pieces >> (16 * k + 13)) & 7u);
    int incl = cnt;
#pragma unroll
    for (int d = 1; d < 64; d <<= 1) {
        const int o = __shfl_up(incl, d);
        if (lane >= d) incl += o;
    }
    const int wave_total = __builtin_amdgcn_readlane(incl, 63);
    if (wave_total == 0) return;
    uint32_t base = 0;
    if (lane == 0) base = atomicAdd(a.n_items, (uint32_t)wave_total);
    base = (uint32_t)__builtin_amdgcn_readfirstlane((int)base);
    uint32_t o = base + (uint32_t)(incl - cnt);
    if (!cnt) return;
    for (int k = 0; k < n_pieces; k++) {
        const uint32_t p = (uint32_t)(pieces >> (16 * k)) & 0xffffu;
        const int nx = (int)((p >> 10) & 7u), ny = (int)((p >> 13) & 7u);
        Rect c = cover, e = exact;
        if (split) {
            const int r0 = (int)(p & 31u), r1 = (int)((p >> 5) & 31u);
            c.x0 = tile_x0 + 8 * r0; c.x1 = imin(tile_x0 + 8 * r1 + 7, tile_x1);
            e.x0 = r0 == 0 ? exact.x0 : c.x0; e.x1 = r1 == ((tile_x1 - tile_x0) >> 3) ? exact.x1 : c.x1;
        }
        const int nb = (c.x1 - c.x0 + 8) >> 3, h = c.y1 - c.y0 + 1;
        const int pb = (nb + nx - 1) / nx, ph = (h + ny - 1) / ny;
        for (int jy = 0; jy < ny; jy++)
            for (int jx = 0; jx < nx; jx++, o++) {
                const int x0 = c.x0 + 8 * pb * jx, x1 = imin(x0 + 8 * pb - 1, c.x1);
                const int y0 = c.y0 + ph * jy, y1 = imin(y0 + ph - 1, c.y1);
                if (o >= a.cap_items) continue;
                a.items[o] = BoxItem::make(image, tile, x0, x1, y0, y1, e.x0, e.x1, e.y0, e.y1);
            }
    }
}

}

__global__ __launch_bounds__(256) void settle_tiles_kernel(BoxArgs a)
{
    if (a.zero8 && blockIdx.x == 0 && threadIdx.x < 8) a.zero8[threadIdx.x] = 0u;
    const int n_all = a.n_clear > a.n_images ? a.n_clear : a.n_images;
    const TileOfThread t = tile_of_thread(a, n_all);
    if (t.valid && !a.dense && t.image < n_all) {
        const uint4 nxt = *(const uint4*)(a.tile_rows_next + 4 * t.idx);
        if (nxt.x <= nxt.y) { *(uint4*)(a.tile_rows_next + 4 * t.idx) = NO_BOX; a.tile_cols_next[t.idx] = 0u; }
    }
    const bool valid = t.valid && t.image < a.n_images;
    const int tile = t.chunk * a.n_strips + t.strip;
    const int tile_r0 = t.chunk * a.rows_per_chunk, tile_r1 = imin(tile_r0 + a.rows_per_chunk, a.H) - 1;
    const int tile_x0 = 240 * t.strip, tile_x1 = imin(tile_x0 + 239, a.W - 1);
    Rect box;
    bool marked = scan_box(a, t, valid, box);
    Rect out{imax(box.x0, tile_x0) & ~7, imin(imin(box.x1, tile_x1) | 7, tile_x1), imax(box.y0, tile_r0), imin(box.y1, tile_r1)};
    if (marked && (out.x0 > out.x1 || out.y0 > out.y1)) marked = false;
    if (!marked) out = {1, 0, 1, 0};
    Rect cover = out, exact = box;
    const bool emits = marked && ((!a.dense && a.cluster) ? cluster_decision(a, t, cover, exact) : true);
    int n_pieces = 0;
    uint64_t pieces = 0;
    bool wide = false, split = false;
    if (marked) {
        int nx, ny;
        const int nb = (cover.x1 - cover.x0 + 8) >> 3, h = cover.y1 - cover.y0 + 1;
        choose_split(nb, h, nx, ny);
        const int limit = ((a.remap_bits >> (t.image % a.cam_mod)) & 1ull) ? a.wide_quads_remap : a.wide_quads_identity;
        const bool own = cover.x0 == out.x0 && cover.x1 == out.x1 && cover.y0 == out.y0 && cover.y1 == out.y1;
        wide = emits && own && a.wide_tiles != nullptr && 2 * nb + 2 * nx >= limit;
        if (wide && a.wide_split && a.wide_bands == 1 && !a.dense) {
            n_pieces = split_at_gaps(a.tile_cols[t.idx], (out.x0 - tile_x0) >> 3, (out.x1 - tile_x0) >> 3, h, limit, pieces);
            split = n_pieces != 0;
            wide = !split;
        }
        if (wide) { out.x0 = tile_x0; out.x1 = tile_x1; cover.x0 = out.x0; cover.x1 = out.x1; }
        else if (emits && !split) { n_pieces = 1; pieces = piece_pack(0, 0, nx, ny); }
    }
    uint32_t prev_x = 1u, prev_y = 1u;
    bool need_clear = valid && record_region(a, t, marked, out, box, prev_x, prev_y);
    if (split && span_first(prev_x) <= span_last(prev_x)) {
        need_clear = true;
        for (int k = 0; k < n_pieces; k++) {
            const uint32_t p = (uint32_t)(pieces >> (16 * k));
            const int x0 = tile_x0 + 8 * (int)(p & 31u), x1 = imin(tile_x0 + 8 * (int)((p >> 5) & 31u) + 7, tile_x1);
            if (x0 <= span_first(prev_x) && span_last(prev_x) <= x1 && out.y0 <= span_first(prev_y) && span_last(prev_y) <= out.y1) need_clear = false;
        }
    }
    clear_previous(a, need_clear, prev_x, prev_y, t.image);
    emit_wide(a, wide, t.image, tile, out.y0, out.y1);
    count_split(a, split);
    emit_items(a, n_pieces, pieces, split, t.image, tile, cover, exact, tile_x0, tile_x1);
}

void launch_settle_tiles(const BoxArgs& a, hipStream_t s)
{
    const int n_all = a.n_clear > a.n_images ? a.n_clear : a.n_images;
    const long long total = (long long)a.n_chunks * a.n_strips * a.cam_mod * ((n_all + a.cam_mod - 1) / a.cam_mod);
    hipLaunchKernelGGL(settle_tiles_kernel, dim3((unsigned)((total + 255) / 256)), dim3(256), 0, s, a);
}

}
```

### mocapv2_amd/csrc/boxes_dev.h

```cpp
#pragma once
#include <hip/hip_runtime.h>
#include <stdint.h>
#include "kernels.h"
#include "bayer.h"
#include "filter_dev.h"

namespace mocap {

namespace {

__device__ __forceinline__ int imin(int a, int b) { return a < b ? a : b; }
__device__ __forceinline__ int imax(int a, int b) { return a > b ? a : b; }
__device__ __forceinline__ int small_div(int n, float rcp_d) { return (int)(((float)n + 0.5f) * rcp_d); }

struct BayerK { int ry, rx; uint32_t cb, cg, cr; int shift; };

struct BayerWin { uint32_t w[9]; };
__device__ __forceinline__ void bayer_win_load(BayerWin& b, const uint8_t* __restrict__ img, int pitch, int W, int H, int x, int y)
{
    const int yc = y < 1 ? 1 : (y > H - 2 ? H - 2 : y);
    const uint32_t xl = (uint32_t)imax(x - 4, 0), xr = (uint32_t)imin(x + 4, W - 4);
#pragma unroll
    for (int r = 0; r < 3; r++) {
        const uint32_t o = (uint32_t)(yc - 1 + r) * (uint32_t)pitch;
        b.w[3 * r] = *(const uint32_t*)(img + o + xl);
        b.w[3 * r + 1] = *(const uint32_t*)(img + o + (uint32_t)x);
        b.w[3 * r + 2] = *(const uint32_t*)(img + o + xr);
    }
}
__device__ __forceinline__ uint32_t bayer_gray4(const BayerWin& b, int W, int H, int x, int y, const BayerK& k)
{
    const int yc = y < 1 ? 1 : (y > H - 2 ? H - 2 : y);
    const bool red_row = (yc & 1) == k.ry;
    const bool eic = (red_row ? k.rx : 1 - k.rx) == 0;
    uint32_t Pc[3], Lc[3], Rc[3], Pg[3];
    uint32_t Lg = 0, Rg = 0;
#pragma unroll
    for (int r = 0; r < 3; r++) {
        const uint32_t pw = b.w[3 * r], w = b.w[3 * r + 1], nw = b.w[3 * r + 2];
        const uint32_t e = prm(0, w, 0x0c020c00u), o = prm(0, w, 0x0c030c01u);
        const uint32_t Le = prm(pw, w, 0x0c010c07u), Ro = prm(nw, w, 0x0c040c02u);
        Pc[r] = eic ? e : o; Lc[r] = eic ? Le : e; Rc[r] = eic ? o : Ro; Pg[r] = eic ? o : e;
        if (r == 1) { Lg = eic ? e : Le; Rg = eic ? Ro : o; }
    }
    const uint32_t cx = red_row ? k.cr : k.cb, cy = red_row ? k.cb : k.cr;
    const LumaCoef kc{cx, k.cg, cy, cx << 16, k.cg << 16, cy << 16, 1u << (k.shift - 1), k.shift};
    uint32_t ca, cb, ga, gb;
    luma2(Pc[1], mean4(Lc[1], Rc[1], Pc[0], Pc[2]), mean4(Lc[0], Rc[0], Lc[2], Rc[2]), kc, ca, cb);
    luma2(mean2(Lg, Rg), Pg[1], mean2(Pg[0], Pg[2]), kc, ga, gb);
    uint32_t g0 = eic ? ca : ga, g1 = eic ? ga : ca, g2 = eic ? cb : gb, g3 = eic ? gb : cb;
    if (x == 0) g0 = g1;
    if (x + 3 == W - 1) g3 = g2;
    return g0 | (g1 << 8) | (g2 << 16) | (g3 << 24);
}
__device__ __forceinline__ uint32_t bayer_gray1(const uint8_t* __restrict__ img, int pitch, int W, int H, int x, int y, const BayerK& k)
{
    const int yc = y < 1 ? 1 : (y > H - 2 ? H - 2 : y), xc = x < 1 ? 1 : (x > W - 2 ? W - 2 : x);
    const uint32_t c = (uint32_t)yc * (uint32_t)pitch + (uint32_t)xc, u = c - (uint32_t)pitch, d = c + (uint32_t)pitch;
    return site_gray(img[c], img[c - 1], img[c + 1], img[u], img[d], img[u - 1], img[u + 1], img[d - 1], img[d + 1], (yc & 1) == k.ry,
                     (xc & 1) == k.rx, k);
}

struct BoxGeom {
    int image, tile, slot, remap;
    int ox0, ox1, oy0, oy1, Q, px0, ty0, ty1, hy0, hy1, PR, ey0, ey1, eq0, eq1;
    bool valid, exact;
};
__device__ __forceinline__ BoxGeom box_geometry(int H, int W, int cam_mod, uint64_t remap_bits, const BoxItem& it)
{
    const uint4 h0 = it.head, h1 = it.box;
    BoxGeom g;
    g.image = uni((int)h0.x); g.tile = uni((int)h0.y);
    g.ox0 = uni(span_first(h0.z)); g.ox1 = uni(span_last(h0.z)); g.oy0 = uni(span_first(h0.w)); g.oy1 = uni(span_last(h0.w));
    const int bx0 = uni(span_first(h1.x)), bx1 = uni(span_last(h1.x)), by0 = uni(span_first(h1.y)), by1 = uni(span_last(h1.y));
    g.valid = g.ox0 <= g.ox1 && g.oy0 <= g.oy1;
    g.slot = g.image % cam_mod;
    g.remap = (int)((remap_bits >> g.slot) & 1ull);
    const int nb = (g.ox1 - g.ox0 + 8) >> 3;
    g.Q = 2 * nb + 2; g.px0 = g.ox0 - 4;
    g.ty0 = imax(g.oy0 - 2, 0); g.ty1 = imin(g.oy1 + 2, H - 1);
    g.hy0 = g.ty0 - 2; g.hy1 = g.ty1 + 2; g.PR = g.hy1 - g.hy0 + 1;
    g.ey0 = imax(imax(by0, g.hy0), 0); g.ey1 = imin(imin(by1, g.hy1), H - 1);
    g.eq0 = imax((imax(bx0, 0) - g.px0) >> 2, 0); g.eq1 = imin((imin(bx1, W - 1) - g.px0) >> 2, g.Q - 1);
    g.exact = g.valid && g.ey0 <= g.ey1 && g.eq0 <= g.eq1;
    return g;
}
struct SrcBounds { int xa, xb, ya, yb; };
__device__ __forceinline__ SrcBounds source_bounds_partial(const ushort4* __restrict__ srcbox, int H, int W, const BoxGeom& g, int lane)
{
    SrcBounds b{0x7fff, -0x8000, 0x7fff, -0x8000};
    if (!g.exact || !g.remap) return b;
    const int ncx8 = (W + 7) >> 3;
    const ushort4* __restrict__ sbx = srcbox + (size_t)g.slot * ncx8 * ((H + 7) >> 3);
    const int cx0 = imax(g.px0 + 4 * g.eq0, 0) >> 3, cx1 = imin(g.px0 + 4 * g.eq1 + 3, W - 1) >> 3, cy0 = g.ey0 >> 3, cy1 = g.ey1 >> 3;
    const int ncw = cx1 - cx0 + 1, ncells = ncw * (cy1 - cy0 + 1);
    const float rcpw = __builtin_amdgcn_rcpf((float)ncw);
    for (int c0 = 0; c0 < ncells; c0 += 64) {
        const int c = imin(c0 + lane, ncells - 1);
        const int cyi = small_div(c, rcpw), cxi = c - cyi * ncw;
        const ushort4 sb = sbx[(cy0 + cyi) * ncx8 + cx0 + cxi];
        b.xa = imin(b.xa, (int)sb.x - 2); b.xb = imax(b.xb, (int)sb.y - 2); b.ya = imin(b.ya, (int)sb.z - 2); b.yb = imax(b.yb, (int)sb.w - 2);
    }
    return b;
}

}

}
```

### mocapv2_amd/csrc/ctx.h

```cpp
#pragma once
#include <hip/hip_runtime.h>
#include <stdint.h>
#include <stdio.h>
#include <stdlib.h>
#include <string.h>
#include <math.h>
#include <string>
#include <vector>
#include <mutex>
#include <memory>
#include "../../include/mocap_hip.h"
#include "kernels.h"

using namespace mocap;

int fail(int code, const char* fmt, ...);

#define HIP_TRY(expr)                                                                                         \
    do {                                                                                                      \
        hipError_t e_ = (expr);                                                                               \
        if (e_ != hipSuccess) return fail(MOCAP_E_HIP, "%s failed: %s", #expr, hipGetErrorString(e_));        \
    } while (0)
#define TRY(expr) do { if (int rc_ = (expr)) return rc_; } while (0)

template <class T, bool Pinned = false>
struct Buf {
    T* p = nullptr;
    size_t n = 0;
    Buf() = default;
    Buf(Buf&& o) : p(o.p), n(o.n) { o.p = nullptr; o.n = 0; }
    Buf& operator=(Buf&& o) { if (this != &o) { release(); p = o.p; n = o.n; o.p = nullptr; o.n = 0; } return *this; }
    ~Buf() { release(); }
    operator T*() const { return p; }
    T* operator->() const { return p; }
    void release()
    {
        if (p) (void)(Pinned ? hipHostFree(p) : hipFree(p));
        p = nullptr; n = 0;
    }
    int reserve(size_t count, bool zero = false)
    {
        if (count <= n) return 0;
        if (p) { HIP_TRY(hipDeviceSynchronize()); release(); }
        HIP_TRY(Pinned ? hipHostMalloc((void**)&p, sizeof(T) * count) : hipMalloc((void**)&p, sizeof(T) * count));
        if (zero) HIP_TRY(hipMemset(p, 0, sizeof(T) * count));
        n = count;
        return 0;
    }
};

struct EvPair { hipEvent_t a, b; };
constexpr size_t PROBE_BYTES = 128 * mocap::PROBE_STRIDE * sizeof(uint32_t);
using mocap::PROBE_STRIDE;

struct SharedComm {
    void* comm = nullptr;
    int rank = 0, world = 1, device = 0;
    hipEvent_t last = nullptr;
    bool have_last = false;
    std::mutex mu;
    bool (*destroy_comm)(void*) = nullptr;
    ~SharedComm()
    {
        if (!comm && !last) return;
        (void)hipSetDevice(device);
        if (last) { if (have_last) (void)hipEventSynchronize(last); (void)hipEventDestroy(last); }
        if (comm && destroy_comm) (void)destroy_comm(comm);
    }
};

struct Tuning {
#define X(name, def, lo, hi) int name = def;
#include "tuning.def"
#undef X
};
#define X(name, def, lo, hi) static_assert((lo) <= (def) && (def) <= (hi), "tuning.def: the default of " #name " lies outside its bounds");
#include "tuning.def"
#undef X

enum ProfSlot { PROF_FILTER, PROF_CONTOURS, PROF_CORRESPOND, PROF_SCAN, PROF_SETTLE, PROF_SLOTS };
static_assert(PROF_SLOTS == 5, "mocap_profile_read hands out five slots");

struct mocap_ctx {
    int device = 0, W = 0, H = 0, n_slots = 0, wpr = 0;
    int box_grid = 2048;
    int n_cu = 256;
    mocap_blob_params prm{5, 5, 255 * 0.85, 500.0, 0.5};
    Tuning tune;
    Buf<uint32_t> maps;
    Buf<uint32_t> map4;
    Buf<ushort4> srcbox;
    Buf<ushort4> rowbox;
    Buf<uint32_t> map_flags;
    Buf<double> lens;
    std::vector<int> slot_state;
    std::vector<int> slot_compact;
    std::vector<uint32_t> slot_wmax;
    Buf<uint2> reach;
    Buf<uint8_t> cflags;
    Buf<uint32_t> mask; size_t mask_images = 0;
    bool mask_dirty = false;
    Buf<uint32_t> cells;
    int last_images = 0;
    Buf<uint32_t> hotmap;
    Buf<uint32_t> tile_rows;
    int tile_rows_flip = 0;
    int tile_rows_hold[2] = {0, 0};
    Buf<uint32_t> tile_cols;
    Buf<uint32_t> cur_box;
    Buf<BoxItem> items;
    Buf<uint4> wide_tiles;
    Buf<uint32_t> n_items;
    hipStream_t side = nullptr; hipEvent_t ev_fork = nullptr, ev_join = nullptr;
    int base_sel = 1; int probe_age = 0; bool probe_pending = false; Buf<uint32_t> probe_dev; Buf<uint32_t, true> probe_host; hipEvent_t probe_ev = nullptr;
    bool walk_count_zeroed = false;
    int probe_images = 0;
    bool hot_dense = false;
    Buf<uint32_t> cells_ext, cur_box_ext; size_t cells_ext_images = 0;
    Buf<uint32_t> mask_out;
    Buf<uint32_t> mask_in;
    Buf<uint8_t> gray_scratch;
    Buf<uint8_t> cwork; size_t cwork_images = 0;
    Buf<uint64_t> walk_list, link_list;
    Buf<uint32_t> walk_count;
    Buf<CameraTable> cams; int n_cam = 0, n_F = 0;
    Buf<double> scratch;
    Buf<double> ba_obj;
    Buf<char> fund_scratch;
    Buf<char> rig_scratch;
    Buf<char> intr_scratch;
    Buf<char, true> ba_pinned;
    std::shared_ptr<struct SharedComm> comm;
    bool profiling = false;
    std::vector<EvPair> ev[PROF_SLOTS];
    std::mutex mu;
};

static int set_device(mocap_ctx* c) { HIP_TRY(hipSetDevice(c->device)); return 0; }

struct Tiling { int rows, n_cgroups, n_strips; };
static Tiling tiling(const mocap_ctx* c)
{
    Tiling t;
    t.rows = c->tune.rows;
    if (c->H < 4 * 32) t.rows = (c->H + 3) / 4 > 8 ? (c->H + 3) / 4 : 8;
    t.n_cgroups = (c->H + 4 * t.rows - 1) / (4 * t.rows);
    t.n_strips = (c->W + 239) / 240;
    return t;
}

static size_t source_cells(const mocap_ctx* c) { return (size_t)((c->H + 7) / 8) * ((c->W + 7) / 8); }
static size_t cells_per_image(const mocap_ctx* c) { Tiling t = tiling(c); return (size_t)t.n_cgroups * 4 * t.n_strips; }
static uint32_t* slot_map(const mocap_ctx* c, int slot) { return c->maps ? c->maps + (size_t)slot * c->H * c->W : nullptr; }
static uint32_t* slot_mapw(const mocap_ctx* c, int slot) { return c->maps ? c->maps + (size_t)(c->n_slots + slot) * c->H * c->W : nullptr; }
static uint32_t* slot_map4(const mocap_ctx* c, int slot) { return c->map4 ? c->map4 + (size_t)slot * c->H * c->W : nullptr; }

struct Carver {
    char* base;
    size_t used = 0;
    template <class T> void take(T*& p, size_t count) { p = base ? (T*)(base + used) : nullptr; used += (sizeof(T) * count + 15) & ~(size_t)15; }
};

void prof_begin(mocap_ctx* c, hipStream_t s, EvPair& p, bool& on);
void prof_end(mocap_ctx* c, ProfSlot slot, hipStream_t s, EvPair& p, bool on);
```

### mocapv2_amd/csrc/kernels.h

```cpp
#pragma once
#include <hip/hip_runtime.h>
#include <stdint.h>

namespace mocap {

__host__ __device__ __forceinline__ uint32_t mask_word_index(int y, int k, int wpr)
{
    return ((uint32_t)(y >> 5) * (uint32_t)wpr + (uint32_t)k) * 32u + (uint32_t)(y & 31);
}
__host__ __device__ __forceinline__ uint32_t mask_byte_index(int y, int b, int wpr)
{
    return mask_word_index(y, b >> 2, wpr) * 4u + (uint32_t)(b & 3);
}
__host__ __device__ __forceinline__ size_t mask_image_words(int H, int wpr) { return (size_t)((H + 31) >> 5) * 32 * (size_t)wpr; }

__device__ __forceinline__ int uni(int v) { return __builtin_amdgcn_readfirstlane(v); }
__device__ __forceinline__ unsigned long long uni64(unsigned long long v)
{
    const unsigned lo = __builtin_amdgcn_readfirstlane((unsigned)v), hi = __builtin_amdgcn_readfirstlane((unsigned)(v >> 32));
    return (unsigned long long)hi << 32 | lo;
}

__device__ __forceinline__ double wave_sum(double v)
{
#pragma unroll
    for (int o = 32; o > 0; o >>= 1) v += __shfl_down(v, o, 64);
    return v;
}
__device__ __forceinline__ double block_sum(double v, double* s_part )
{
    v = wave_sum(v);
    __syncthreads();
    if ((threadIdx.x & 63) == 0) s_part[threadIdx.x >> 6] = v;
    __syncthreads();
    return (s_part[0] + s_part[1]) + (s_part[2] + s_part[3]);
}

void launch_mask_convert(const uint32_t* src, uint32_t* dst, int n_images, int H, int wpr, bool to_blocked, hipStream_t s);

struct FilterArgs {
    const uint8_t* src;
    size_t image_stride;
    int pitch, H, W;
    uint32_t* mask;
    int words_per_row;
    uint32_t* cells;
    const uint32_t* map;
    const uint32_t* mapw;
    const uint4* tiles; const uint32_t* n_tiles; uint32_t cap_tiles;
    int pipelined;
    int cam_mod;
    int n_images, n_steps;
    int thr_mul;
    int rows_per_chunk, n_strips, n_cgroups;
    int staged = 0;
    const uint32_t* map4 = nullptr;
    const ushort4* rowbox = nullptr;
    int stage_dw = 0;
};
void launch_rowbox(const uint32_t* map4, ushort4* rowbox, int H, int W, int n_strips, hipStream_t s);
int rows_stage_dwords();
void launch_filter_rows_staged(const FilterArgs& a, bool list, int blocks, hipStream_t s);

struct BayerArgs {
    const uint8_t* src; uint8_t* dst;
    int H, W, n_images;
    long spitch, dpitch;
    size_t sstride, dstride;
    int ry, rx;
    uint32_t cb, cg, cr;
    int shift;
};

#ifndef MOCAP_BOX_HCAP
#define MOCAP_BOX_HCAP 1536
#define MOCAP_BOX_SCAP 6656
#define MOCAP_BOX_MAX_PARTS 4
#endif
constexpr int BOX_HCAP = MOCAP_BOX_HCAP;
constexpr int BOX_SCAP = MOCAP_BOX_SCAP;
constexpr int BOX_MAX_PARTS = MOCAP_BOX_MAX_PARTS;
constexpr int SPLIT_COUNTER = 12;
__host__ __device__ __forceinline__ uint32_t span_pack(int a, int b) { return (uint32_t)a | ((uint32_t)b << 16); }
__host__ __device__ __forceinline__ int span_first(uint32_t s) { return (int)(s & 0xffffu); }
__host__ __device__ __forceinline__ int span_last(uint32_t s) { return (int)(s >> 16); }
struct BoxItem {
    uint4 head, box;
    static __device__ __forceinline__ BoxItem make(int image, int tile, int x0, int x1, int y0, int y1, int bx0, int bx1, int by0, int by1)
    {
        const bool empty = x0 > x1 || y0 > y1;
        return {make_uint4((uint32_t)image, (uint32_t)tile, empty ? 1u : span_pack(x0, x1), span_pack(y0, y1)),
                make_uint4(span_pack(bx0, bx1), span_pack(by0, by1), 0u, 0u)};
    }
};
static_assert(sizeof(BoxItem) == 32, "two 16-byte halves");
__host__ __device__ __forceinline__ uint4 tile_box_pack(uint32_t out_x, uint32_t out_y, int bx0, int bx1, int by0, int by1)
{
    return make_uint4(out_x, out_y, span_pack(bx0, bx1), span_pack(by0, by1));
}
struct WideTile { int image, tile, y0, y1; };
__host__ __device__ __forceinline__ uint4 wide_tile_pack(int image, int tile, int y0, int y1)
{
    return make_uint4((uint32_t)image, (uint32_t)tile, (uint32_t)y0, (uint32_t)(y0 <= y1 ? y1 : y0 - 1));
}
__host__ __device__ __forceinline__ WideTile wide_tile_unpack(uint4 e) { return {(int)e.x, (int)e.y, (int)e.z, (int)e.w}; }

struct BoxArgs {
    const uint8_t* src; size_t image_stride; int pitch, H, W;
    uint32_t* mask; int words_per_row;
    uint32_t* cells;
    const uint32_t* map4;
    const ushort4* srcbox;
    uint64_t remap_bits;
    int cam_mod, n_images, n_steps;
    int thr_mul;
    int rows_per_chunk, n_strips, n_chunks;
    uint32_t* tile_rows;
    uint32_t* tile_rows_next;
    const uint32_t* tile_cols;
    uint32_t* tile_cols_next;
    int wide_split;
    int n_clear;
    int cluster;
    uint32_t* cur_box;
    BoxItem* items; uint32_t* n_items; uint32_t cap_items;
    uint64_t* timing;
    int prio;
    int stage_bytes;
    uint4* wide_tiles;
    uint32_t cap_wide; int wide_quads_remap, wide_quads_identity, wide_bands;
    uint32_t* zero8;
    int dense;
    int ext_mask;
    BayerArgs bayer;
};
void launch_settle_tiles(const BoxArgs& a, hipStream_t s);
void launch_box_filter(const BoxArgs& a, int grid, hipStream_t s, bool bayer = false);
int box_filter_blocks_per_cu();
void launch_srcbox(const uint32_t* map4, ushort4* srcbox, int H, int W, hipStream_t s);

struct MapArgs {
    double K[9], dist[5];
    int H, W;
    uint32_t* map;
    uint32_t* mapw;
    uint32_t* map4;
    uint32_t* flags;
};

struct ContourRec {
    int32_t key;
    int32_t is_hole;
    int32_t sx, sy;
    int32_t npts;
    int32_t steps;
    int64_t a00, a10, a01;
    double area, perimeter;
    int32_t kept, cx, cy;
    int32_t link;
    int32_t parent;
    int32_t order;
};

struct ContourArgs {
    const uint32_t* mask;
    int words_per_row, H, W, n_images;
    int32_t* out_xy;
    int32_t* out_count;
    long xy_stride, count_stride;
    int max_blobs;
    double min_area, min_circ;
    ContourRec* dbg;
    int32_t* dbg_count;
    int dbg_cap;
    int max_steps;
    const uint32_t* cells;
    const uint32_t* boxes;
    int rows_per_chunk, n_chunks, n_strips;
    uint64_t* timing;
    void* work;
    int prio;
    uint64_t* walk_list;
    uint64_t* link_list;
    uint32_t* walk_count;
    uint32_t* wait_list;
    int follow_grid;
    int follow_grid2;
    int counters_zeroed;
    int defer_links;
    int image_grid;
    int follow_list;
    int tree_pass;
    uint64_t* follow_dbg;
    int follow_dbg_list;
};

enum { BLOB_ERR_CANDIDATES = -2, BLOB_ERR_CONTOURS = -3, BLOB_ERR_STEPS = -4, BLOB_ERR_DEPTH = -5 };

void launch_filter_mask(const FilterArgs& a, bool remap, hipStream_t s);
void launch_filter_tiles(const FilterArgs& a, bool remap, int blocks, hipStream_t s);
constexpr int PROBE_STRIDE = 32;
struct BrightArgs {
    const uint8_t* src; size_t image_stride; int pitch, H, W, n_images;
    int cam_mod;
    uint32_t ncx_magic;
    int wide;
    int base;
    int hot, hot_edge, hot_corner;
    const uint2* reach;
    const uint8_t* cflags;
    uint32_t* tile_rows; int n_chunks, n_strips; uint32_t rows_magic;
    uint32_t* mask; size_t mask_words; int mask_aligned16;
    uint32_t* probe; int base_alt, hot_alt;
    int prio;
    int max_blocks;
    uint32_t* block_ctr;
    int blocks_x;
    int slices;
    int image0, slice_images;
    uint32_t* hotmap;
    int hot_words;
    uint32_t* zero_counters;
    int mark_grid;
    uint32_t* tile_cols;
};
int hot_map_words(int H, int W, int wide);
void launch_mark_tiles(const BrightArgs& a, hipStream_t s);
void launch_bright_cells(const BrightArgs& a, hipStream_t s);
struct StatArgs { const uint32_t* map; const uint32_t* mapw; uint32_t* acc; uint32_t* stats; int H, W; uint32_t* edge; int* reach; };
void launch_remap_stats(const StatArgs& a, hipStream_t s);
void launch_undistort_map(const MapArgs& m, hipStream_t s);
void launch_contours(const ContourArgs& a, hipStream_t s);
void launch_contour_follow(const ContourArgs& a, int grid, hipStream_t s);
size_t contour_work_bytes();
size_t contour_walk_bytes();
size_t contour_link_bytes();
void launch_box_blur(const uint8_t* src, uint8_t* dst, int H, int W, int sp, int dp, int ksize, hipStream_t s);
void launch_undistort(const uint8_t* src, uint8_t* dst, int H, int W, int sp, int dp, const uint32_t* map, const uint32_t* mapw,
                      hipStream_t s);
void launch_mask_expand(const uint32_t* mask, int wpr, uint8_t* dst, int H, int W, int dp, hipStream_t s);
void launch_median5(const uint8_t* src, uint8_t* dst, int H, int W, int sp, int dp, int ithresh, int apply, hipStream_t s);
void launch_demosaic(const uint8_t* bayer, uint8_t* bgr, int H, int W, int sp, hipStream_t s);
void launch_bayer_gray(const BayerArgs& a, hipStream_t s);
bool bayer_scan_fusable(const BayerArgs& a);
bool bayer_scan_direct(const BayerArgs& a);
void launch_bayer_gray_scan(const BayerArgs& a, const BrightArgs& b, hipStream_t s);

struct CameraTable {
    double K[32][9], dist[32][5], R[32][9], t[32][3];
    double F[31][9];
    int n_cam, n_F;
};

struct CorrArgs {
    const CameraTable* cams;
    const void* pts;
    const int32_t* counts;
    long pt_st, pt_sc, cnt_st, cnt_sc;
    int pts_f64;
    int T, C, P;
    double cutoff;
    int max_groups;
    double* root_xyz;
    double* root_err;
    double* root_grp;
    int32_t* root_idx;
    int32_t* order;
    int32_t* n_roots;
    int prio;
    int threads;
    double* scratch;
    int step_budget;
    int lds_budget;
};

struct VisArgs {
    const CameraTable* cams;
    const void* pts;
    const int32_t* counts;
    long pt_st, pt_sc, cnt_st, cnt_sc;
    int pts_f64;
    int T, C, P;
    int distorted;
    double cutoff, gate2, max_err;
    int min_views, max_passes;
    int max_hyp;
    int Q;
    double* xyz;
    double* err;
    int32_t* idx;
    uint32_t* views;
    int32_t* n;
    unsigned char* scratch;
    size_t step_bytes;
    int lds_budget;
};

struct TriArgs {
    const CameraTable* cams;
    const double* pts;
    const uint8_t* valid;
    int N, C;
    int compact_k;
    double* xyz;
    int32_t* ok;
};

struct ReprojArgs {
    const CameraTable* cams;
    const double* pts;
    const uint8_t* valid;
    const double* xyz;
    int N, C, compact_k;
    double* mse;
    int32_t* ok;
};

struct EpiArgs {
    const CameraTable* cams;
    const void* roots;
    const void* cand;
    int n_roots, n_cand, pts_f64, f_index;
    double* dist;
    float* lines;
};

struct BaArgs {
    const CameraTable* cams;
    const double* params;
    const double* pts;
    const uint8_t* valid;
    int N, C, B;
    double* obj;
    float* res;
    int32_t* counts;
};

struct FundArgs {
    const double* pts_a;
    const double* pts_b;
    const int32_t* offset;
    const int32_t* samples;
    int n_pairs, H, max_n;
    double thr2;
    double* F_all;
    int32_t* counts;
    int32_t* pair_err;
    double* F_sample;
    double* F_refit;
    uint8_t* inlier;
    int32_t* status;
};

struct LmState {
    double lambda, nu;
    double cost, cost0;
    int32_t stop, status;
    int32_t iters, cur;
    int32_t chol_fail, chol_fail_prev, behind, trial_behind;
};

struct RigState : LmState {
    double t1_norm;
    int32_t layout_err, pad;
};
enum { RIG_LIN_COST = 0, RIG_PRED_CAM = 1, RIG_NORM2_CAM = 2, RIG_N_SCALARS = 4 };
enum { RIG_STOP_MAX_ITERS = 1, RIG_STOP_FTOL = 2, RIG_STOP_LAMBDA = 3, RIG_STOP_CHOLESKY = 4, RIG_ERR_LAYOUT = -2, RIG_ERR_BEHIND = -3 };

struct RigArgs {
    const CameraTable* cams;
    const int32_t* obs_offset;
    const int32_t* obs_cam;
    const double* obs_uv;
    int C, N, n_obs;
    int n_pairs, n_lin_blocks, n_chunks;
    int loss;
    double loss_c2;
    double* poses_io;
    double* points_io;
    RigState* state;
    double* poses;
    double* points;
    uint32_t* mask;
    double* W;
    double* Vinv;
    double* vdiag;
    double* gp;
    double* lin_part;
    double* cost_part;
    double* schur_part;
    double* S;
    double* rhs;
    double* gc;
    double* udiag;
    double* chol;
    double* delta_c;
    double* upd_part;
    double* scalars;
    double* history;
    double* result;
    double* obs_err;
    double* obs_weight;
};

void launch_rig_init(const RigArgs& a, double lambda0, hipStream_t s);
void launch_rig_linearize(const RigArgs& a, hipStream_t s);
void launch_rig_iteration(const RigArgs& a, int it, int max_iters, double ftol, hipStream_t s);
void launch_rig_finish(const RigArgs& a, hipStream_t s);
void launch_rig_residuals(const RigArgs& a, hipStream_t s);
int rig_lin_blocks(int N);
int rig_schur_chunks(int N);

constexpr int SELFCAL_P = 15;
constexpr int SELFCAL_U = 120 + SELFCAL_P;
constexpr int SELFCAL_BLK = SELFCAL_P * SELFCAL_P + SELFCAL_P;
struct SelfcalArgs {
    const int32_t* obs_offset;
    const int32_t* obs_cam;
    const double* obs_uv;
    int C, N, n_obs;
    int n_pairs, n_lin_blocks, n_chunks;
    int schur_chunk;
    int loss;
    double loss_c2;
    double* kd_io;
    double* poses_io;
    double* points_io;
    const int32_t* free_cols;
    int32_t* cam_count;
    RigState* state;
    double* kd;
    double* poses;
    double* points;
    uint32_t* mask;
    double* W;
    double* Vinv;
    double* vdiag;
    double* gp;
    double* lin_part;
    double* cost_part;
    double* schur_part;
    double* S;
    double* rhs;
    double* gc;
    double* udiag;
    double* chol;
    double* delta_c;
    double* upd_part;
    double* scalars;
    double* history;
    double* result;
    double* obs_err;
    double* obs_weight;
};
void launch_selfcal_init(const SelfcalArgs& a, double lambda0, hipStream_t s);
void launch_selfcal_linearize(const SelfcalArgs& a, hipStream_t s);
void launch_selfcal_iteration(const SelfcalArgs& a, int it, int max_iters, double ftol, hipStream_t s);
void launch_selfcal_finish(const SelfcalArgs& a, hipStream_t s);
void launch_selfcal_residuals(const SelfcalArgs& a, hipStream_t s);
int selfcal_lin_blocks(int N);
int selfcal_schur_chunk(int N);

using IntrState = LmState;
enum { INTR_ERR_LAYOUT = -2, INTR_ERR_BEHIND = -3, INTR_ERR_DEGENERATE = -4 };
enum { INTR_REC_SUMS = 0, INTR_REC_T = 136, INTR_REC_YG = 181, INTR_REC_L = 190, INTR_REC = 216 };

struct IntrArgs {
    int n_cams, n_views;
    const int32_t* view_offset;
    const int32_t* point_offset;
    const int32_t* view_cam;
    const int32_t* image_size;
    const int32_t* cam_bad;
    const double* obj;
    const double* img;
    double* kd_io;
    double* poses_io;
    double* view_rms;
    double* history;
    double* result;
    int32_t* lin_status;
    int max_iters;
    IntrState* state;
    double* kd;
    double* poses;
    double* view_cost;
    double* H;
    double* rec;
    double* gv;
    double* S;
    double* rhs;
    double* gc;
    double* udiag;
    double* delta_c;
    double* lin_cost;
    double* cam_part;
    double* upd_part;
};
void launch_intr_begin(const IntrArgs& a, int have_start, double lambda0, hipStream_t s);
void launch_intr_linearize(const IntrArgs& a, int it, bool solve, hipStream_t s);
void launch_intr_iteration(const IntrArgs& a, int it, double ftol, hipStream_t s);
void launch_intr_finish(const IntrArgs& a, hipStream_t s);

enum { CORR_ERR_GROUPS = -2, CORR_ERR_TRUNCATED = -3, CORR_ERR_BLOB = -4, CORR_ERR_OUTPUT = -5 };
enum { FUND_ERR_SAMPLE = -2, FUND_ERR_DEGENERATE = -3 };
enum { TRACK_ERR_FULL = -2, TRACK_ERR_IDS = -3, TRACK_ERR_INPUT = -4, TRACK_ERR_COUNT = -5 };

constexpr int TRACK_MAX = 256;
struct TrackHeader { int32_t next_id, reserved0; int64_t steps; int64_t reserved[6]; };
struct TrackSlot { double pos[3], vel[3]; int32_t id, miss, hits, alive; };
static_assert(sizeof(TrackHeader) == 64 && sizeof(TrackSlot) == 64, "the state buffer's layout is part of the ABI");
struct TrackArgs {
    const double* xyz;
    const int32_t* n;
    int T, Q, M;
    void* state;
    double gate, beta;
    int max_miss;
    int32_t* id;
    int32_t* slot;
    int32_t* age;
    int32_t* status;
};
void launch_track_markers(const TrackArgs& a, hipStream_t s);

enum { RIGID_LOST = 1, RIGID_ERR_BLIND = -2, RIGID_ERR_CAPACITY = -3, RIGID_ERR_MODEL = -4, RIGID_ERR_HYP = -5 };
constexpr int RIGID_MAX_DET = 64;
constexpr int RIGID_MAX_MARKERS = 8;
constexpr int RIGID_MAX_TRIPLES = 56;
constexpr int RIGID_MAX_BODIES = 16;
constexpr int RIGID_MAX_HYP = 4096;
struct RigidArgs {
    const double* xyz;
    const int32_t* n;
    int T, Q, B;
    const double* model;
    const int32_t* n_markers;
    const int32_t* tri;
    const int32_t* n_tri;
    double tol, gate;
    int min_markers, max_hyp;
    double* R;
    double* t;
    double* q;
    double* rms;
    int32_t* n_in;
    int32_t* label;
    int32_t* status;
};
void launch_rigid_poses(const RigidArgs& a, hipStream_t s);

enum { SUBPIX_EMPTY = 1, SUBPIX_EDGE = 2, SUBPIX_NEIGHBOUR = 4, SUBPIX_MOVING = 8, SUBPIX_CUT = 16 };
constexpr int SUBPIX_MAX_BLOBS = 256;
constexpr int SUBPIX_LENS = 16;
struct RefineArgs {
    const uint8_t* src; size_t image_stride; int pitch, H, W;
    int n_images, cam_mod;
    int bayer, ry, rx; uint32_t cb, cg, cr; int shift;
    const double* lens;
    const int32_t* xy; long xy_stride;
    const int32_t* count; long count_stride;
    int max_blobs;
    int radius, floor, iters, coords;
    double* out_xy; long out_xy_stride;
    int32_t* out_info; long out_info_stride;
};
void launch_refine_centroids(const RefineArgs& a, hipStream_t s);

void launch_fundamental_ransac(const FundArgs& a, hipStream_t s);

enum { LDS_USER_CORRESPOND, LDS_USER_VISIBLE, LDS_USERS };
int workgroup_lds_limit(int user, const void* kernel_f64, const void* kernel_i32);
void launch_correspond(const CorrArgs& a, hipStream_t s);
size_t correspond_smem_bytes(int P, int C);
bool correspond_fits(int P, int C);
void launch_correspond_visible(const VisArgs& a, hipStream_t s);
size_t correspond_visible_smem_bytes(int P, int C);
bool correspond_visible_fits(int P, int C);
size_t correspond_visible_step_bytes(int C, int max_hyp);
void launch_epipolar_scores(const EpiArgs& a, hipStream_t s);
void launch_ba_residuals(const BaArgs& a, hipStream_t s);
void launch_triangulate(const TriArgs& a, hipStream_t s);
void launch_reproject(const ReprojArgs& a, hipStream_t s);

}
```

### mocapv2_amd/csrc/scan_mark.h

```cpp
#pragma once
#include <hip/hip_runtime.h>
#include <stdint.h>
#include "kernels.h"

namespace mocap {

__device__ __forceinline__ uint32_t excess2_row(uint32_t lo, uint32_t hi, uint32_t base4, uint32_t c8)
{
    uint32_t s = __builtin_amdgcn_sad_u8(lo, base4, 0u);
    s = __builtin_amdgcn_sad_u8(lo, 0u, s);
    s = __builtin_amdgcn_sad_u8(hi, base4, s);
    s = __builtin_amdgcn_sad_u8(hi, 0u, s);
    return s - c8;
}

__device__ __forceinline__ uint32_t tile_col_bits(int st, int xa, int xb)
{
    const int x0 = 240 * st, ca = xa > x0 ? xa - x0 : 0, cb = xb - x0 < 239 ? xb - x0 : 239;
    return (2u << (cb >> 3)) - (1u << (ca >> 3));
}

__device__ __forceinline__ void widen_tile_boxes(const BrightArgs& a, const uint2 rc, uint32_t* __restrict__ rows, uint32_t* __restrict__ cols)
{
    const int x0 = (int)(rc.x & 0xffffu), x1 = (int)(rc.x >> 16), y0 = (int)(rc.y & 0xffffu), y1 = (int)(rc.y >> 16);
    if (x0 > x1) return;
    const int xa = x0 - 4 > 0 ? x0 - 4 : 0, xb = x1 + 4 < a.W - 1 ? x1 + 4 : a.W - 1;
    const int ya = y0 - 4 > 0 ? y0 - 4 : 0, yb = y1 + 4 < a.H - 1 ? y1 + 4 : a.H - 1;
    const int ch0 = (int)(((uint32_t)ya * a.rows_magic) >> 23), ch1 = (int)(((uint32_t)yb * a.rows_magic) >> 23);
    const int st0 = (int)(((uint32_t)xa * 34953u) >> 23), st1 = (int)(((uint32_t)xb * 34953u) >> 23);
    for (int ch = ch0; ch <= ch1; ch++)
        for (int st = st0; st <= st1; st++) {
            const int t = ch * a.n_strips + st;
            const uint32_t m = tile_col_bits(st, xa, xb);
            const uint4 cur = *(const uint4*)(rows + 4 * t);
            const uint32_t have = cols[t];
            if (!(cur.x <= (uint32_t)ya && cur.y >= (uint32_t)yb && cur.z <= (uint32_t)xa && cur.w >= (uint32_t)xb)) {
                atomicMin(&rows[4 * t], (uint32_t)ya);
                atomicMax(&rows[4 * t + 1], (uint32_t)yb);
                atomicMin(&rows[4 * t + 2], (uint32_t)xa);
                atomicMax(&rows[4 * t + 3], (uint32_t)xb);
            }
            if ((have & m) != m) atomicOr(&cols[t], m);
        }
}

__device__ __forceinline__ void mark_hot_cell(const BrightArgs& a, const uint2* __restrict__ reach, const uint8_t* __restrict__ cflags,
                                              uint32_t* __restrict__ rows, uint32_t* __restrict__ cols, int ci, uint32_t acc)
{
    if ((int)acc > a.hot_corner) {
        const uint2 rc = reach[ci];
        const uint32_t fl = cflags[ci];
        if ((int)acc > ((fl & 2u) ? a.hot_corner : (fl & 1u) ? a.hot_edge : a.hot)) widen_tile_boxes(a, rc, rows, cols);
    }
}

__device__ __forceinline__ uint32_t hot_level(const BrightArgs& a, uint32_t acc)
{
    return (uint32_t)((int)acc > a.hot_corner) + (uint32_t)((int)acc > a.hot_edge) + (uint32_t)((int)acc > a.hot);
}
__device__ __forceinline__ bool level_is_hot(uint32_t level, uint32_t fl)
{
    return level >= ((fl & 2u) ? 1u : (fl & 1u) ? 2u : 3u);
}

}
```

Baseline: 406,100 frames/s.

## Merge tile column bitmask into tile box record as 4-pixel quad bits

Drops the separate tile_cols array. Each tile record now stores the row min/max plus a 64-bit mask of covered 4-pixel column quads (with a small margin). That mask takes the place of the x min/max and the old 8-pixel column bits. The settle kernel rebuilds the x range and the gap-split bytes from that mask. This removes one atomic target, one load and one clear per tile. Each atomic is now issued only when its own field would change. A reciprocal-based divide replaces the integer division in the mask-clear loop. X extents become coarser (quad granularity), which may widen boxes slightly.

```diff
diff --git a/mocapv2_amd/csrc/abi_blob.hip b/mocapv2_amd/csrc/abi_blob.hip
--- a/mocapv2_amd/csrc/abi_blob.hip
+++ b/mocapv2_amd/csrc/abi_blob.hip
@@ -102,7 +102,7 @@
     auto t5 = [](int n) { return (n - 1 < 2 ? n - 1 : 2) + 1; };
     auto t5full = [](int n) { return n < 5 ? n : 5; };
     const long long per_tap = 1024LL * (2LL * thr_mul - 2LL * b.base - 1), per_tap_alt = 1024LL * (2LL * thr_mul - 2LL * b.base_alt - 1);
-    if (!c->tile_rows || !c->tile_cols || !c->reach || !c->cflags) ok = false;
+    if (!c->tile_rows || !c->reach || !c->cflags) ok = false;
     if (ok && wmax > 0 && per_tap > 0) {
         b.allow = (int)((per_tap * t5full(c->W) * t5full(c->H) - 1) / wmax);
         const long long taps1 = t5(c->W) * t5full(c->H) < t5full(c->W) * t5(c->H) ? t5(c->W) * t5full(c->H) : t5full(c->W) * t5(c->H);
@@ -185,8 +185,6 @@
     a.tile_rows = c->tile_rows + (c->tile_rows_flip ? tr_words : 0);
     a.tile_rows_next = c->tile_rows + (c->tile_rows_flip ? 0 : tr_words);
     a.n_clear = c->tile_rows_hold[c->tile_rows_flip ^ 1];
-    a.tile_cols = c->tile_cols + (c->tile_rows_flip ? tr_words / 4 : 0);
-    a.tile_cols_next = c->tile_cols + (c->tile_rows_flip ? 0 : tr_words / 4);
     a.wide_split = c->tune.wide_split == 2 || (c->tune.wide_split == 1 && !c->hot_dense);
     a.cluster = c->tune.cluster;
     a.cur_box = bt.own_mask ? c->cur_box : c->cur_box_ext;
@@ -202,8 +200,7 @@
     return a;
 }
 
-static BrightArgs bright_args(const mocap_ctx* c, const Batch& bt, const FilterPath& p, const ScanBounds& sb, uint32_t* tile_rows, uint32_t* tile_cols,
-                              bool scan_zeroes)
+static BrightArgs bright_args(const mocap_ctx* c, const Batch& bt, const FilterPath& p, const ScanBounds& sb, uint32_t* tile_rows, bool scan_zeroes)
 {
     const Tiling tl = tiling(c);
     uint64_t ncx64 = (uint64_t)((c->W + 7) / 8);
@@ -222,15 +219,13 @@
     b.zero_counters = scan_zeroes ? c->n_items.p : nullptr;
     b.block_ctr = c->n_items + 160;
     b.slices = c->tune.scan_slices; b.image0 = 0; b.slice_images = bt.n_images;
-    b.tile_cols = tile_cols;
     return b;
 }
 
-static int scan_tiles(mocap_ctx* c, const Batch& bt, const FilterPath& p, const ScanBounds& sb, uint32_t* tile_rows, uint32_t* tile_cols,
-                      bool scan_zeroes, BrightArgs& b, bool& mark_after_scan)
+static int scan_tiles(mocap_ctx* c, const Batch& bt, const FilterPath& p, const ScanBounds& sb, uint32_t* tile_rows, bool scan_zeroes, BrightArgs& b, bool& mark_after_scan)
 {
     const hipStream_t s = bt.s;
-    b = bright_args(c, bt, p, sb, tile_rows, tile_cols, scan_zeroes);
+    b = bright_args(c, bt, p, sb, tile_rows, scan_zeroes);
     const bool probe = sb.fixed_base < 0 && !c->probe_pending && sb.allow_alt >= 0 && sb.base_alt != sb.base && !p.bayer &&
                        (c->probe_age == 0 || c->probe_age >= 32);
     if (probe) {
@@ -372,7 +367,7 @@
     a.zero8 = bt.own_mask ? c->walk_count.p : nullptr;
     c->walk_count_zeroed = a.zero8 != nullptr;
     BrightArgs mark_args{}; bool mark_after_scan = false;
-    if (!a.dense) TRY(scan_tiles(c, bt, p, sb, a.tile_rows, const_cast<uint32_t*>(a.tile_cols), scan_zeroes, mark_args, mark_after_scan));
+    if (!a.dense) TRY(scan_tiles(c, bt, p, sb, a.tile_rows, scan_zeroes, mark_args, mark_after_scan));
     else if (p.bayer) {
         launch_bayer_gray(p.bl, s);
         HIP_TRY(hipGetLastError());
@@ -502,13 +497,11 @@
     const size_t tiles = n_images * cells_per_image(c);
     TRY(c->mask.reserve(n_images * mask_image_words(c->H, c->wpr), true));
     TRY(c->cells.reserve(tiles, true));
-    std::vector<uint32_t> init(tiles * 4);
-    for (size_t i = 0; i < init.size(); i += 2) { init[i] = 0xffffffffu; init[i + 1] = 0u; }
+    std::vector<uint32_t> init(tiles * 4, 0u);
+    for (size_t i = 0; i < init.size(); i += 4) init[i] = 0xffffffffu;
     TRY(c->tile_rows.reserve(2 * init.size()));
     HIP_TRY(hipMemcpy(c->tile_rows, init.data(), sizeof(uint32_t) * init.size(), hipMemcpyHostToDevice));
     HIP_TRY(hipMemcpy(c->tile_rows + init.size(), init.data(), sizeof(uint32_t) * init.size(), hipMemcpyHostToDevice));
-    TRY(c->tile_cols.reserve(2 * tiles));
-    HIP_TRY(hipMemset(c->tile_cols, 0, sizeof(uint32_t) * 2 * tiles));
     const int hw0 = hot_map_words(c->H, c->W, 0), hw1 = hot_map_words(c->H, c->W, 1);
     TRY(c->hotmap.reserve(n_images * (hw0 > hw1 ? hw0 : hw1), true));
     for (size_t i = 0; i < init.size(); i++) init[i] = 1u;
@@ -526,7 +519,7 @@
     if ((size_t)n_images <= c->mask_images) return 0;
     c->mask_images = 0; c->last_images = 0;
     if (int rc = grow_mask_group(c, n_images)) {
-        c->mask.release(); c->cells.release(); c->tile_rows.release(); c->tile_cols.release(); c->hotmap.release(); c->cur_box.release();
+        c->mask.release(); c->cells.release(); c->tile_rows.release(); c->hotmap.release(); c->cur_box.release();
         c->items.release(); c->wide_tiles.release();
         return rc;
     }
diff --git a/mocapv2_amd/csrc/bayer_gray.hip b/mocapv2_amd/csrc/bayer_gray.hip
--- a/mocapv2_amd/csrc/bayer_gray.hip
+++ b/mocapv2_amd/csrc/bayer_gray.hip
@@ -184,11 +184,10 @@
         const int slot = image % b.cam_mod;
         const uint2* __restrict__ reach = b.reach + (size_t)slot * n;
         const uint8_t* __restrict__ cflags = b.cflags + (size_t)slot * n;
-        uint32_t* __restrict__ rows = b.tile_rows + (size_t)image * b.n_chunks * b.n_strips * 4;
-        uint32_t* __restrict__ cols = b.tile_cols + (size_t)image * b.n_chunks * b.n_strips;
+        uint32_t* __restrict__ rec = b.tile_rows + (size_t)image * b.n_chunks * b.n_strips * 4;
         const int ci = cy * ncx + (x0 >> 3);
-        mark_hot_cell(b, reach, cflags, rows, cols, ci, acc0);
-        mark_hot_cell(b, reach, cflags, rows, cols, ci + 1, acc1);
+        mark_hot_cell(b, reach, cflags, rec, ci, acc0);
+        mark_hot_cell(b, reach, cflags, rec, ci + 1, acc1);
     }
 }
 
diff --git a/mocapv2_amd/csrc/blob_scan.hip b/mocapv2_amd/csrc/blob_scan.hip
--- a/mocapv2_amd/csrc/blob_scan.hip
+++ b/mocapv2_amd/csrc/blob_scan.hip
@@ -69,8 +69,7 @@
     const int slot = image % a.cam_mod;
     const uint2* __restrict__ reach = a.reach + (size_t)slot * n;
     const uint8_t* __restrict__ cflags = a.cflags + (size_t)slot * n;
-    uint32_t* __restrict__ rows = a.tile_rows + (size_t)image * a.n_chunks * a.n_strips * 4;
-    uint32_t* __restrict__ cols = a.tile_cols + (size_t)image * a.n_chunks * a.n_strips;
+    uint32_t* __restrict__ rec = a.tile_rows + (size_t)image * a.n_chunks * a.n_strips * 4;
     const uint32_t base4 = (uint32_t)a.base * 0x01010101u, c8 = 8u * (uint32_t)a.base;
     uint32_t level[2] = {0u, 0u}, sum[2];
 #pragma unroll
@@ -106,8 +105,8 @@
         }
     }
     if (!MAP) {
-        mark_hot_cell(a, reach, cflags, rows, cols, ci[0], sum[0]);
-        mark_hot_cell(a, reach, cflags, rows, cols, ci[1], sum[1]);
+        mark_hot_cell(a, reach, cflags, rec, ci[0], sum[0]);
+        mark_hot_cell(a, reach, cflags, rec, ci[1], sum[1]);
     }
     if (MAP) {
         const int lane = threadIdx.x & 63;
@@ -135,7 +134,7 @@
 __global__ __launch_bounds__(256) void mark_tiles_kernel(BrightArgs a)
 {
     __shared__ uint16_t s_list[4][1024];
-    __shared__ uint32_t s_tab[4][32][6];
+    __shared__ uint32_t s_tab[4][32][5];
     const int lane = threadIdx.x & 63, wv = threadIdx.x >> 6;
     const int wpi = (a.hot_words + 255) >> 8;
     const int n_cells = ((a.W + 7) >> 3) * ((a.H + 7) >> 3);
@@ -152,23 +151,18 @@
 #pragma unroll
     for (int k = 0; k < 4; k++)
         if (wk[k] != 0u) hm[wave_word0 + 64 * k + lane] = 0u;
-    uint32_t (*tab)[6] = s_tab[wv];
-    if (lane < 32) { tab[lane][0] = 0xffffffffu; tab[lane][1] = 0xffffffffu; tab[lane][2] = 0u; tab[lane][3] = 0xffffffffu; tab[lane][4] = 0u; tab[lane][5] = 0u; }
+    uint32_t (*tab)[5] = s_tab[wv];
+    if (lane < 32) { tab[lane][0] = 0xffffffffu; tab[lane][1] = 0xffffffffu; tab[lane][2] = 0u; tab[lane][3] = 0u; tab[lane][4] = 0u; }
     const int slot = image % a.cam_mod;
     const uint2* __restrict__ reach = a.reach + (size_t)slot * n_cells;
     const uint8_t* __restrict__ cflags = a.cflags + (size_t)slot * n_cells;
-    uint32_t* __restrict__ rows = a.tile_rows + (size_t)image * a.n_chunks * a.n_strips * 4;
-    uint32_t* __restrict__ cols = a.tile_cols + (size_t)image * a.n_chunks * a.n_strips;
-    auto widen = [&](int t, uint32_t ya, uint32_t yb, uint32_t xa, uint32_t xb, uint32_t m) __attribute__((always_inline)) {
-        const uint4 cur = *(const uint4*)(rows + 4 * t);
-        const uint32_t have = cols[t];
-        if (!(cur.x <= ya && cur.y >= yb && cur.z <= xa && cur.w >= xb)) {
-            atomicMin(&rows[4 * t], ya);
-            atomicMax(&rows[4 * t + 1], yb);
-            atomicMin(&rows[4 * t + 2], xa);
-            atomicMax(&rows[4 * t + 3], xb);
-        }
-        if ((have & m) != m) atomicOr(&cols[t], m);
+    uint32_t* __restrict__ rec = a.tile_rows + (size_t)image * a.n_chunks * a.n_strips * 4;
+    auto widen = [&](int t, uint32_t ya, uint32_t yb, uint32_t mlo, uint32_t mhi) __attribute__((always_inline)) {
+        const uint4 cur = *(const uint4*)(rec + 4 * t);
+        if (cur.x > ya) atomicMin(&rec[4 * t], ya);
+        if (cur.y < yb) atomicMax(&rec[4 * t + 1], yb);
+        if ((cur.z & mlo) != mlo) atomicOr(&rec[4 * t + 2], mlo);
+        if ((cur.w & mhi) != mhi) atomicOr(&rec[4 * t + 3], mhi);
     };
 #pragma unroll 1
     for (int k = 0; k < 4; k++) {
@@ -207,14 +201,15 @@
                         for (int ch = ch0; ch <= ch1; ch++)
                             for (int st = st0; st <= st1; st++) {
                                 const int t = ch * a.n_strips + st, q = t & 31;
-                                const uint32_t m = tile_col_bits(st, xa, xb);
+                                const uint64_t m = tile_quad_bits(st, xa, xb);
+                                const uint32_t mlo = (uint32_t)m, mhi = (uint32_t)(m >> 32);
                                 const uint32_t old = atomicCAS(&tab[q][0], 0xffffffffu, (uint32_t)t);
                                 if (old == 0xffffffffu || old == (uint32_t)t) {
                                     atomicMin(&tab[q][1], (uint32_t)ya); atomicMax(&tab[q][2], (uint32_t)yb);
-                                    atomicMin(&tab[q][3], (uint32_t)xa); atomicMax(&tab[q][4], (uint32_t)xb);
-                                    atomicOr(&tab[q][5], m);
+                                    if (mlo) atomicOr(&tab[q][3], mlo);
+                                    if (mhi) atomicOr(&tab[q][4], mhi);
                                 } else
-                                    widen(t, (uint32_t)ya, (uint32_t)yb, (uint32_t)xa, (uint32_t)xb, m);
+                                    widen(t, (uint32_t)ya, (uint32_t)yb, mlo, mhi);
                             }
                     }
                 }
@@ -223,7 +218,7 @@
         __builtin_amdgcn_s_waitcnt(0xc07f);
         __builtin_amdgcn_wave_barrier();
     }
-    if (lane < 32 && tab[lane][0] != 0xffffffffu) widen((int)tab[lane][0], tab[lane][1], tab[lane][2], tab[lane][3], tab[lane][4], tab[lane][5]);
+    if (lane < 32 && tab[lane][0] != 0xffffffffu) widen((int)tab[lane][0], tab[lane][1], tab[lane][2], tab[lane][3], tab[lane][4]);
     __builtin_amdgcn_s_waitcnt(0xc07f);
     __builtin_amdgcn_wave_barrier();
     }
diff --git a/mocapv2_amd/csrc/blob_settle.hip b/mocapv2_amd/csrc/blob_settle.hip
--- a/mocapv2_amd/csrc/blob_settle.hip
+++ b/mocapv2_amd/csrc/blob_settle.hip
@@ -29,7 +29,14 @@
 namespace {
 
 struct Rect { int x0, x1, y0, y1; };
-constexpr uint4 NO_BOX = {0xffffffffu, 0u, 0xffffffffu, 0u};
+constexpr uint4 NO_BOX = {0xffffffffu, 0u, 0u, 0u};
+
+__device__ __forceinline__ Rect record_box(uint4 rec, int st, int W)
+{
+    Rect b{0, 0, (int)rec.x, (int)rec.y};
+    tile_quad_columns(st, (uint64_t)rec.w << 32 | rec.z, W, b.x0, b.x1);
+    return b;
+}
 
 struct TileOfThread { int image, chunk, strip; size_t idx; bool valid; };
 __device__ __forceinline__ TileOfThread tile_of_thread(const BoxArgs& a, int n_all)
@@ -50,13 +57,15 @@
     return t;
 }
 
-__device__ __forceinline__ bool scan_box(const BoxArgs& a, const TileOfThread& t, bool valid, Rect& box)
+__device__ __forceinline__ bool scan_box(const BoxArgs& a, const TileOfThread& t, bool valid, Rect& box, uint64_t& quads)
 {
     box = {0, a.W - 1, 0, a.H - 1};
+    quads = 0;
     if (!valid || a.dense) return valid;
     const uint4 raw = *(const uint4*)(a.tile_rows + 4 * t.idx);
     if (raw.x > raw.y) return false;
-    box = {(int)raw.z, (int)raw.w, (int)raw.x, (int)raw.y};
+    quads = (uint64_t)raw.w << 32 | raw.z;
+    box = record_box(raw, t.strip, a.W);
     return true;
 }
 
@@ -72,7 +81,8 @@
         if (o.x > o.y) continue;
         if (first < 0) first = k;
         n_marked++;
-        u.y0 = imin(u.y0, (int)o.x); u.y1 = imax(u.y1, (int)o.y); u.x0 = imin(u.x0, (int)o.z); u.x1 = imax(u.x1, (int)o.w);
+        const Rect ob = record_box(o, sx, a.W);
+        u.y0 = imin(u.y0, ob.y0); u.y1 = imax(u.y1, ob.y1); u.x0 = imin(u.x0, ob.x0); u.x1 = imax(u.x1, ob.x1);
     }
     if (n_marked < 2) return true;
     const int bx_lo = 240 * s0, bx_hi = imin(240 * (s0 + 2) - 1, a.W - 1), by_lo = c0 * a.rows_per_chunk, by_hi = imin((c0 + 2) * a.rows_per_chunk, a.H) - 1;
@@ -111,8 +121,9 @@
         const int x0 = span_first(cx), x1 = span_last(cx), y0 = span_first(cy), y1 = span_last(cy);
         uint8_t* m = (uint8_t*)(a.mask + (size_t)cimage * mask_image_words(a.H, a.words_per_row));
         const int b0 = x0 >> 3, nr = y1 - y0 + 1, n = nr * ((x1 >> 3) - b0 + 1);
+        const float rcp_nr = __builtin_amdgcn_rcpf((float)nr);
         for (int i = lane; i < n; i += 64) {
-            const int bc = i / nr;
+            const int bc = small_div(i, rcp_nr);
             m[mask_byte_index(y0 + (i - bc * nr), b0 + bc, a.words_per_row)] = 0;
         }
     }
@@ -212,14 +223,15 @@
     const TileOfThread t = tile_of_thread(a, n_all);
     if (t.valid && !a.dense && t.image < n_all) {
         const uint4 nxt = *(const uint4*)(a.tile_rows_next + 4 * t.idx);
-        if (nxt.x <= nxt.y) { *(uint4*)(a.tile_rows_next + 4 * t.idx) = NO_BOX; a.tile_cols_next[t.idx] = 0u; }
+        if (nxt.x <= nxt.y) *(uint4*)(a.tile_rows_next + 4 * t.idx) = NO_BOX;
     }
     const bool valid = t.valid && t.image < a.n_images;
     const int tile = t.chunk * a.n_strips + t.strip;
     const int tile_r0 = t.chunk * a.rows_per_chunk, tile_r1 = imin(tile_r0 + a.rows_per_chunk, a.H) - 1;
     const int tile_x0 = 240 * t.strip, tile_x1 = imin(tile_x0 + 239, a.W - 1);
     Rect box;
-    bool marked = scan_box(a, t, valid, box);
+    uint64_t quads;
+    bool marked = scan_box(a, t, valid, box, quads);
     Rect out{imax(box.x0, tile_x0) & ~7, imin(imin(box.x1, tile_x1) | 7, tile_x1), imax(box.y0, tile_r0), imin(box.y1, tile_r1)};
     if (marked && (out.x0 > out.x1 || out.y0 > out.y1)) marked = false;
     if (!marked) out = {1, 0, 1, 0};
@@ -236,7 +248,7 @@
         const bool own = cover.x0 == out.x0 && cover.x1 == out.x1 && cover.y0 == out.y0 && cover.y1 == out.y1;
         wide = emits && own && a.wide_tiles != nullptr && 2 * nb + 2 * nx >= limit;
         if (wide && a.wide_split && a.wide_bands == 1 && !a.dense) {
-            n_pieces = split_at_gaps(a.tile_cols[t.idx], (out.x0 - tile_x0) >> 3, (out.x1 - tile_x0) >> 3, h, limit, pieces);
+            n_pieces = split_at_gaps(tile_quad_bytes(quads), (out.x0 - tile_x0) >> 3, (out.x1 - tile_x0) >> 3, h, limit, pieces);
             split = n_pieces != 0;
             wide = !split;
         }
diff --git a/mocapv2_amd/csrc/boxes_dev.h b/mocapv2_amd/csrc/boxes_dev.h
--- a/mocapv2_amd/csrc/boxes_dev.h
+++ b/mocapv2_amd/csrc/boxes_dev.h
@@ -11,7 +11,6 @@
 
 __device__ __forceinline__ int imin(int a, int b) { return a < b ? a : b; }
 __device__ __forceinline__ int imax(int a, int b) { return a > b ? a : b; }
-__device__ __forceinline__ int small_div(int n, float rcp_d) { return (int)(((float)n + 0.5f) * rcp_d); }
 
 struct BayerK { int ry, rx; uint32_t cb, cg, cr; int shift; };
 
diff --git a/mocapv2_amd/csrc/ctx.h b/mocapv2_amd/csrc/ctx.h
--- a/mocapv2_amd/csrc/ctx.h
+++ b/mocapv2_amd/csrc/ctx.h
@@ -106,7 +106,6 @@
     Buf<uint32_t> tile_rows;
     int tile_rows_flip = 0;
     int tile_rows_hold[2] = {0, 0};
-    Buf<uint32_t> tile_cols;
     Buf<uint32_t> cur_box;
     Buf<BoxItem> items;
     Buf<uint4> wide_tiles;
diff --git a/mocapv2_amd/csrc/kernels.h b/mocapv2_amd/csrc/kernels.h
--- a/mocapv2_amd/csrc/kernels.h
+++ b/mocapv2_amd/csrc/kernels.h
@@ -20,6 +20,8 @@
     const unsigned lo = __builtin_amdgcn_readfirstlane((unsigned)v), hi = __builtin_amdgcn_readfirstlane((unsigned)(v >> 32));
     return (unsigned long long)hi << 32 | lo;
 }
+
+__device__ __forceinline__ int small_div(int n, float rcp_d) { return (int)(((float)n + 0.5f) * rcp_d); }
 
 __device__ __forceinline__ double wave_sum(double v)
 {
@@ -84,6 +86,34 @@
 __host__ __device__ __forceinline__ uint32_t span_pack(int a, int b) { return (uint32_t)a | ((uint32_t)b << 16); }
 __host__ __device__ __forceinline__ int span_first(uint32_t s) { return (int)(s & 0xffffu); }
 __host__ __device__ __forceinline__ int span_last(uint32_t s) { return (int)(s >> 16); }
+__host__ __device__ __forceinline__ uint64_t tile_quad_bits(int st, int xa, int xb)
+{
+    const int base = 240 * st - 4;
+    const int qa = xa > base ? (xa - base) >> 2 : 0, qb = xb - base < 248 ? (xb - base) >> 2 : 61;
+    return (2ull << qb) - (1ull << qa);
+}
+__host__ __device__ __forceinline__ void tile_quad_columns(int st, uint64_t m, int W, int& x0, int& x1)
+{
+    const uint32_t lo = (uint32_t)m, hi = (uint32_t)(m >> 32);
+#if defined(__HIP_DEVICE_COMPILE__)
+    const int q0 = lo ? __ffs((int)lo) - 1 : 31 + __ffs((int)hi), q1 = hi ? 63 - __clz((int)hi) : 31 - __clz((int)lo);
+#else
+    const int q0 = lo ? __builtin_ctz(lo) : 32 + __builtin_ctz(hi), q1 = hi ? 63 - __builtin_clz(hi) : 31 - __builtin_clz(lo);
+#endif
+    const int base = 240 * st - 4, a = base + 4 * q0, b = base + 4 * q1 + 3;
+    x0 = a > 0 ? a : 0; x1 = b < W - 1 ? b : W - 1;
+}
+__host__ __device__ __forceinline__ uint32_t tile_quad_bytes(uint64_t m)
+{
+    uint64_t v = ((m | (m >> 1)) >> 1) & 0x0555555555555555ull;
+    v = (v | (v >> 1)) & 0x3333333333333333ull;
+    v = (v | (v >> 2)) & 0x0f0f0f0f0f0f0f0full;
+    v = (v | (v >> 4)) & 0x00ff00ff00ff00ffull;
+    v = (v | (v >> 8)) & 0x0000ffff0000ffffull;
+    v = (v | (v >> 16)) & 0x00000000ffffffffull;
+    return (uint32_t)v;
+}
+
 struct BoxItem {
     uint4 head, box;
     static __device__ __forceinline__ BoxItem make(int image, int tile, int x0, int x1, int y0, int y1, int bx0, int bx1, int by0, int by1)
@@ -117,8 +147,6 @@
     int rows_per_chunk, n_strips, n_chunks;
     uint32_t* tile_rows;
     uint32_t* tile_rows_next;
-    const uint32_t* tile_cols;
-    uint32_t* tile_cols_next;
     int wide_split;
     int n_clear;
     int cluster;
@@ -222,7 +250,6 @@
     int hot_words;
     uint32_t* zero_counters;
     int mark_grid;
-    uint32_t* tile_cols;
 };
 int hot_map_words(int H, int W, int wide);
 void launch_mark_tiles(const BrightArgs& a, hipStream_t s);
diff --git a/mocapv2_amd/csrc/scan_mark.h b/mocapv2_amd/csrc/scan_mark.h
--- a/mocapv2_amd/csrc/scan_mark.h
+++ b/mocapv2_amd/csrc/scan_mark.h
@@ -14,13 +14,7 @@
     return s - c8;
 }
 
-__device__ __forceinline__ uint32_t tile_col_bits(int st, int xa, int xb)
-{
-    const int x0 = 240 * st, ca = xa > x0 ? xa - x0 : 0, cb = xb - x0 < 239 ? xb - x0 : 239;
-    return (2u << (cb >> 3)) - (1u << (ca >> 3));
-}
-
-__device__ __forceinline__ void widen_tile_boxes(const BrightArgs& a, const uint2 rc, uint32_t* __restrict__ rows, uint32_t* __restrict__ cols)
+__device__ __forceinline__ void widen_tile_boxes(const BrightArgs& a, const uint2 rc, uint32_t* __restrict__ rec)
 {
     const int x0 = (int)(rc.x & 0xffffu), x1 = (int)(rc.x >> 16), y0 = (int)(rc.y & 0xffffu), y1 = (int)(rc.y >> 16);
     if (x0 > x1) return;
@@ -31,26 +25,23 @@
     for (int ch = ch0; ch <= ch1; ch++)
         for (int st = st0; st <= st1; st++) {
             const int t = ch * a.n_strips + st;
-            const uint32_t m = tile_col_bits(st, xa, xb);
-            const uint4 cur = *(const uint4*)(rows + 4 * t);
-            const uint32_t have = cols[t];
-            if (!(cur.x <= (uint32_t)ya && cur.y >= (uint32_t)yb && cur.z <= (uint32_t)xa && cur.w >= (uint32_t)xb)) {
-                atomicMin(&rows[4 * t], (uint32_t)ya);
-                atomicMax(&rows[4 * t + 1], (uint32_t)yb);
-                atomicMin(&rows[4 * t + 2], (uint32_t)xa);
-                atomicMax(&rows[4 * t + 3], (uint32_t)xb);
-            }
-            if ((have & m) != m) atomicOr(&cols[t], m);
+            const uint64_t m = tile_quad_bits(st, xa, xb);
+            const uint32_t mlo = (uint32_t)m, mhi = (uint32_t)(m >> 32);
+            const uint4 cur = *(const uint4*)(rec + 4 * t);
+            if (cur.x > (uint32_t)ya) atomicMin(&rec[4 * t], (uint32_t)ya);
+            if (cur.y < (uint32_t)yb) atomicMax(&rec[4 * t + 1], (uint32_t)yb);
+            if ((cur.z & mlo) != mlo) atomicOr(&rec[4 * t + 2], mlo);
+            if ((cur.w & mhi) != mhi) atomicOr(&rec[4 * t + 3], mhi);
         }
 }
 
 __device__ __forceinline__ void mark_hot_cell(const BrightArgs& a, const uint2* __restrict__ reach, const uint8_t* __restrict__ cflags,
-                                              uint32_t* __restrict__ rows, uint32_t* __restrict__ cols, int ci, uint32_t acc)
+                                              uint32_t* __restrict__ rec, int ci, uint32_t acc)
 {
     if ((int)acc > a.hot_corner) {
         const uint2 rc = reach[ci];
         const uint32_t fl = cflags[ci];
-        if ((int)acc > ((fl & 2u) ? a.hot_corner : (fl & 1u) ? a.hot_edge : a.hot)) widen_tile_boxes(a, rc, rows, cols);
+        if ((int)acc > ((fl & 2u) ? a.hot_corner : (fl & 1u) ? a.hot_edge : a.hot)) widen_tile_boxes(a, rc, rec);
     }
 }
 
```

Result: faster. 437,200 frames/s, median of 6 (+7.7%).
